# cfdeinza/reinforcement-learning-rendezvous

Measured on NVIDIA B200. Metric: env-steps/sec, higher is better.
Workload: dtype f64

## Files before the change

reinforcement_learning_rendezvous_b200/_native.py:

```python
from __future__ import annotations

import ctypes as C
import importlib.util
import os
import shutil
import subprocess
import sysconfig

PKG_DIR = os.path.dirname(os.path.abspath(__file__))
CSRC_DIR = os.path.join(PKG_DIR, "csrc")
INCLUDE_DIR = os.path.join(os.path.dirname(PKG_DIR), "include")
LIB_PATH = os.environ.get("RDV_B200_LIB") or os.path.join(CSRC_DIR, "librdv_b200.so")
HOST_SRC = os.path.join(CSRC_DIR, "rdv_host.c")
HOST_LIB = os.path.join(PKG_DIR, "_rdv_host" + (sysconfig.get_config_var("EXT_SUFFIX") or ".so"))
SOURCES = ("rdv_b200.cu",)
HEADERS = ("rdv_math.cuh", "rdv_env.cuh", "rdv_step.cuh", "rdv_policy.cuh", "rdv_policy_tc.cuh")

ABI_VERSION = 15
OBS_DIM, ACT_DIM, N_UNIFORMS = 17, 6, 24

(RCX, RCY, RCZ, VCX, VCY, VCZ, QCW, QCX, QCY, QCZ, WCX, WCY, WCZ, QTW, QTX, QTY, QTZ, WTX, WTY, WTZ,
 TDV, TDW, EPRET, NF64) = range(24)
I_STEP, I_SUCCESS, I_COLLIDED, I_EPISODE, NI32 = range(5)
STAT_NAMES = ("steps", "episodes", "return_sum", "length_sum", "succeeded", "collided", "delta_v_sum",
              "delta_w_sum", "end_obs", "end_time", "end_bubble", "end_attitude", "reward_sum",
              "rk_accepted", "rk_rejected", "failures")
NSTATS = len(STAT_NAMES)
EP_RETURN, EP_LENGTH, EP_SUCCESS, EP_COLLIDED, EP_DELTA_V, EP_DELTA_W, EP_NCOL = range(7)
INTEGRATOR_RK45, INTEGRATOR_CLOSED_FORM = 0, 1
END_REASONS = ("obs", "time", "bubble", "attitude")


class RdvParams(C.Structure):
    _fields_ = [
        ("rc0", C.c_double * 3), ("vc0", C.c_double * 3), ("qc0", C.c_double * 4),
        ("wc0", C.c_double * 3), ("qt0", C.c_double * 4), ("wt0", C.c_double * 3),
        ("rc0_range", C.c_double), ("vc0_range", C.c_double), ("qc0_range", C.c_double),
        ("wc0_range", C.c_double), ("qt0_range", C.c_double), ("wt0_range", C.c_double),
        ("koz_radius", C.c_double), ("corridor_half_angle", C.c_double), ("h", C.c_double),
        ("dt", C.c_double), ("t_max", C.c_double),
        ("collision_coef", C.c_double), ("bonus_coef", C.c_double), ("fuel_coef", C.c_double),
        ("att_coef", C.c_double),
        ("inertia_c", C.c_double * 9), ("inertia_t", C.c_double * 9),
        ("torque_c", C.c_double * 3),
        ("integrator", C.c_int32), ("reserved0", C.c_int32),
        ("inv_inertia_c", C.c_double * 9), ("inv_inertia_t", C.c_double * 9),
        ("max_delta_v", C.c_double), ("max_delta_w", C.c_double), ("max_axial_distance", C.c_double),
        ("max_axial_speed", C.c_double), ("max_wc", C.c_double),
        ("max_attitude_error", C.c_double), ("max_rd_error", C.c_double), ("max_vd_error", C.c_double),
        ("max_qd_error", C.c_double), ("max_wd_error", C.c_double),
        ("rd", C.c_double * 3), ("capture_axis", C.c_double * 3), ("corridor_axis", C.c_double * 3),
        ("bubble0", C.c_double), ("bubble_rate", C.c_double), ("bubble_min", C.c_double), ("n", C.c_double),
        ("cw", C.c_double * 17),
        ("max_delta_v_f32", C.c_float), ("fuel_num_f32", C.c_float), ("fuel_den_f32", C.c_float),
        ("iso_c", C.c_int32), ("iso_t", C.c_int32), ("done_steps", C.c_int32),
        ("inv_max_attitude_error", C.c_double), ("inv_max_rd_error", C.c_double), ("inv_max_qd_error", C.c_double),
        ("koz_radius_sq", C.c_double), ("max_rd_error_sq", C.c_double), ("max_vd_error_sq", C.c_double),
        ("max_wd_error_sq", C.c_double),
        ("fuel_scale", C.c_double),
        ("att_scale", C.c_double), ("bonus_scale", C.c_double), ("collision_scale", C.c_double),
        ("obs_inv_r", C.c_double), ("obs_inv_v", C.c_double), ("obs_inv_w", C.c_double),
        ("near_sq", C.c_double),
        ("box_hi_r", C.c_int32), ("box_hi_v", C.c_int32), ("box_hi_w", C.c_int32), ("reserved1", C.c_int32),
    ]


class RdvState(C.Structure):
    _fields_ = [("f64", C.c_void_p), ("i32", C.c_void_p), ("ld", C.c_int64), ("param_table", C.c_void_p),
                ("param_block", C.c_void_p)]


class RdvStepIO(C.Structure):
    _fields_ = [
        ("actions", C.c_void_p), ("act_f64", C.c_int32), ("auto_reset", C.c_int32),
        ("obs", C.c_void_p), ("reward", C.c_void_p), ("done", C.c_void_p),
        ("terminal_obs", C.c_void_p), ("end_reason", C.c_void_p), ("episode_record", C.c_void_p),
        ("stats", C.c_void_p),
        ("reward_f32", C.c_void_p), ("fin_count", C.c_void_p), ("fin_rows", C.c_void_p),
        ("fin_capacity", C.c_int32), ("fin_append", C.c_int32), ("fin_env_base", C.c_int32), ("reserved", C.c_int32),
    ]


class RdvFinishedRow(C.Structure):
    _fields_ = [("env", C.c_int32), ("end_reason", C.c_int32), ("terminal_obs", C.c_float * 17), ("pad", C.c_float),
                ("record", C.c_double * 6)]


class RdvPolicy(C.Structure):
    _fields_ = [
        ("w0", C.c_void_p), ("b0", C.c_void_p), ("w1", C.c_void_p), ("b1", C.c_void_p),
        ("w2", C.c_void_p), ("b2", C.c_void_p), ("hidden", C.c_int32), ("reserved", C.c_int32),
        ("log_std", C.c_void_p),
    ]


class RdvRolloutIO(C.Structure):
    _fields_ = [
        ("steps", C.c_int32), ("action_source", C.c_int32), ("auto_reset", C.c_int32), ("reserved", C.c_int32),
        ("actions", C.c_void_p), ("action_seed", C.c_uint64), ("step_base", C.c_int64),
        ("actions_out", C.c_void_p), ("obs", C.c_void_p), ("rewards", C.c_void_p), ("dones", C.c_void_p),
        ("obs_steps", C.c_void_p), ("stats", C.c_void_p), ("policy", RdvPolicy),
        ("reset_rows", C.c_void_p), ("sm_reserve", C.c_int32), ("reserved2", C.c_int32), ("mc_out", C.c_void_p),
    ]


RESET_ROWS = 23
(MC_EP_LEN, MC_NUM_COLLISIONS, MC_COLLIDED, MC_TOTAL_REWARD, MC_TOTAL_DELTA_V, MC_NUM_SUCCESSES, MC_SUCCEEDED,
 MC_MIN_KOZ, MC_POS_ERR, MC_VEL_ERR, MC_ATT_ERR, MC_ROT_ERR, MC_LEVEL, MC_TAIL_COUNT, MC_END_REASON,
 MC_TOTAL_DELTA_W, MC_NCOL) = range(17)
TUNE_ROLLOUT_TPB, TUNE_RESET_REFILL, TUNE_ROLLOUT_PDL, TUNE_ROLLOUT_HELPERS = 0, 1, 2, 3


ACTIONS_F32, ACTIONS_F64, ACTIONS_PHILOX, ACTIONS_POLICY, ACTIONS_POLICY_SAMPLE = 0, 1, 2, 3, 4


PROTOTYPES = {
    "rdv_abi_version": (C.c_int, []),
    "rdv_sizeof_params": (C.c_int, []),
    "rdv_sizeof": (C.c_int, [C.c_int]),
    "rdv_strerror": (C.c_char_p, [C.c_int]),
    "rdv_tune": (C.c_int, [C.c_int, C.c_int]),
    "rdv_params_default": (None, [C.POINTER(RdvParams)]),
    "rdv_params_derive": (C.c_int, [C.POINTER(RdvParams)]),
    "rdv_step": (C.c_int, [C.POINTER(RdvParams), C.POINTER(RdvState), C.POINTER(RdvStepIO), C.c_int64,
                           C.c_uint64, C.c_int64, C.c_void_p]),
    "rdv_rollout": (C.c_int, [C.POINTER(RdvParams), C.POINTER(RdvState), C.POINTER(RdvRolloutIO), C.c_int64,
                              C.c_uint64, C.c_int64, C.c_void_p]),
    "rdv_reset": (C.c_int, [C.POINTER(RdvParams), C.POINTER(RdvState), C.c_void_p, C.c_void_p, C.c_void_p,
                            C.c_int64, C.c_uint64, C.c_int64, C.c_int, C.c_void_p]),
    "rdv_observe": (C.c_int, [C.POINTER(RdvParams), C.POINTER(RdvState), C.c_void_p, C.c_int64, C.c_void_p]),
    "rdv_errors": (C.c_int, [C.POINTER(RdvParams), C.POINTER(RdvState), C.c_void_p, C.c_void_p, C.c_void_p,
                             C.c_void_p, C.c_int64, C.c_void_p]),
    "rdv_refresh_flags": (C.c_int, [C.POINTER(RdvParams), C.POINTER(RdvState), C.c_int64, C.c_void_p]),
    "rdv_frame_transform": (C.c_int, [C.c_void_p, C.c_void_p, C.c_void_p, C.c_int64, C.c_int, C.c_void_p]),
    "rdv_policy_forward": (C.c_int, [C.POINTER(RdvPolicy), C.c_void_p, C.c_void_p, C.c_int64, C.c_void_p]),
    "rdv_policy_forward_ffma": (C.c_int, [C.POINTER(RdvPolicy), C.c_void_p, C.c_void_p, C.c_int64, C.c_void_p]),
    "rdv_math_probe": (C.c_int, [C.c_void_p, C.c_void_p, C.c_int64, C.c_int, C.c_void_p]),
    "rdv_fp64_peak_probe": (C.c_int, [C.c_void_p, C.c_int, C.c_int, C.c_int, C.c_void_p]),
}

_lib = None


def nvcc_command(out=LIB_PATH):
    nvcc = shutil.which("nvcc") or "/usr/local/cuda/bin/nvcc"
    return [nvcc, "-gencode", "arch=compute_100a,code=sm_100a", "-lineinfo", "-O3", "-std=c++17",
            "-I", INCLUDE_DIR, "-shared", "-Xcompiler", "-fPIC", "-o", out] + \
           [os.path.join(CSRC_DIR, s) for s in SOURCES]


def is_stale():
    if not os.path.exists(LIB_PATH):
        return True
    t = os.path.getmtime(LIB_PATH)
    deps = [os.path.join(CSRC_DIR, f) for f in SOURCES + HEADERS] + [os.path.join(INCLUDE_DIR, "rdv_b200.h")]
    return any(os.path.getmtime(d) > t for d in deps if os.path.exists(d))


def build_host(force=False):
    global _host
    if force or not os.path.exists(HOST_LIB) or os.path.getmtime(HOST_LIB) < os.path.getmtime(HOST_SRC):
        cc = shutil.which("gcc") or shutil.which("cc") or "gcc"
        import numpy
        subprocess.run([cc, "-O2", "-fPIC", "-shared", "-Wall", "-I", sysconfig.get_paths()["include"],
                        "-I", numpy.get_include(), "-o", HOST_LIB, HOST_SRC], check=True)
        _host = None
    return HOST_LIB


_host = None


def host():
    global _host
    if _host is None:
        if not os.path.exists(HOST_LIB):
            raise RuntimeError(f"{HOST_LIB} is missing: build it with `python -c 'import __graft_entry__ as g; g.build()'`")
        spec = importlib.util.spec_from_file_location("_rdv_host", HOST_LIB)
        mod = importlib.util.module_from_spec(spec)
        spec.loader.exec_module(mod)
        _host = mod
    return _host


def build(force=False, verbose=False):
    global _lib
    build_host(force=force)
    if force or is_stale():
        cmd = nvcc_command()
        if verbose:
            cmd = cmd[:1] + ["-Xptxas", "-v"] + cmd[1:]
            print(" ".join(cmd))
        subprocess.run(cmd, check=True)
        _lib = None
    return LIB_PATH


def lib():
    global _lib
    if _lib is None:
        if not os.path.exists(LIB_PATH):
            raise RuntimeError(
                f"{LIB_PATH} is missing: build it with `python -c 'import __graft_entry__ as g; g.build()'` "
                "(nvcc, sm_100a).  This package has no CPU fallback.")
        L = C.CDLL(LIB_PATH)
        for name, (res, args) in PROTOTYPES.items():
            fn = getattr(L, name)
            fn.restype, fn.argtypes = res, args
        if L.rdv_abi_version() != ABI_VERSION:
            raise RuntimeError(f"librdv_b200.so ABI {L.rdv_abi_version()} != binding ABI {ABI_VERSION}; rebuild")
        for which, mirror in enumerate((RdvParams, RdvState, RdvStepIO, RdvRolloutIO, RdvPolicy, RdvFinishedRow)):
            if L.rdv_sizeof(which) != C.sizeof(mirror):
                raise RuntimeError(f"{mirror.__name__} layout mismatch between include/rdv_b200.h "
                                   f"({L.rdv_sizeof(which)} B) and _native.py ({C.sizeof(mirror)} B)")
        _lib = L
    return _lib


def strerror(status: int) -> str:
    return lib().rdv_strerror(int(status)).decode()


def check(status: int, what: str):
    if status != 0:
        raise RuntimeError(f"{what} failed: {strerror(status)} (status {status})")
```

reinforcement_learning_rendezvous_b200/csrc/rdv_b200.cu:

```cuda
#include <cuda_runtime.h>
#include <math.h>
#include <string.h>
#include <stdlib.h>
#include <atomic>
#include <mutex>
#include "rdv_step.cuh"
#include "rdv_policy.cuh"
#include "rdv_policy_tc.cuh"

namespace rdv {


RDV_DEV double warp_sum(double v)
{
#pragma unroll
    for (int o = 16; o > 0; o >>= 1) v += __shfl_xor_sync(0xffffffffu, v, o);
    return v;
}

struct StepStats {
    unsigned steps, episodes, succeeded, collided, end0, end1, end2, end3, rk_acc, rk_rej, fail;
    double ep_return, ep_length, delta_v, delta_w, reward;
};

template <int NWARPS>
RDV_DEV void reduce_stats(const StepStats &st, double *g_stats, double (*s_stats)[RDV_NSTATS])
{
    const unsigned full = 0xffffffffu;
    const int lane = threadIdx.x & 31, warp = threadIdx.x >> 5;
    double v[RDV_NSTATS];
    v[RDV_S_STEPS] = (double)__reduce_add_sync(full, st.steps);
    v[RDV_S_EPISODES] = (double)__reduce_add_sync(full, st.episodes);
    v[RDV_S_RK_ACCEPTED] = (double)__reduce_add_sync(full, st.rk_acc);
    v[RDV_S_RK_REJECTED] = (double)__reduce_add_sync(full, st.rk_rej);
    v[RDV_S_FAILURES] = (double)__reduce_add_sync(full, st.fail);
    v[RDV_S_REWARD] = warp_sum(st.reward);
    const bool any_done = v[RDV_S_EPISODES] > 0.0;
    if (any_done) {
        v[RDV_S_SUCCEEDED] = (double)__reduce_add_sync(full, st.succeeded);
        v[RDV_S_COLLIDED] = (double)__reduce_add_sync(full, st.collided);
#pragma unroll
        for (int k = 0; k < 4; ++k) v[RDV_S_END_OBS + k] = (double)__reduce_add_sync(full, (k==0?st.end0:k==1?st.end1:k==2?st.end2:st.end3));
        v[RDV_S_RETURN] = warp_sum(st.ep_return);
        v[RDV_S_LENGTH] = warp_sum(st.ep_length);
        v[RDV_S_DELTA_V] = warp_sum(st.delta_v);
        v[RDV_S_DELTA_W] = warp_sum(st.delta_w);
    } else {
        v[RDV_S_SUCCEEDED] = v[RDV_S_COLLIDED] = v[RDV_S_RETURN] = v[RDV_S_LENGTH] = 0.0;
        v[RDV_S_DELTA_V] = v[RDV_S_DELTA_W] = 0.0;
#pragma unroll
        for (int k = 0; k < 4; ++k) v[RDV_S_END_OBS + k] = 0.0;
    }
    if (lane == 0) {
#pragma unroll
        for (int k = 0; k < RDV_NSTATS; ++k) s_stats[warp][k] = v[k];
    }
    __syncthreads();
    if (threadIdx.x < RDV_NSTATS) {
        double acc = 0.0;
#pragma unroll
        for (int w = 0; w < NWARPS; ++w) acc += s_stats[w][threadIdx.x];
        if (acc != 0.0) atomicAdd(g_stats + threadIdx.x, acc);
    }
}

template <bool TABLE>
RDV_DEV const RdvParams &params_of(const RdvParams &Pc, const RdvState &S, const int64_t env)
{
    if constexpr (TABLE) return S.param_table[S.param_block[env >> 5]];
    else return Pc;
}

RDV_DEV double pair_swap(double v) { return __shfl_xor_sync(0xffffffffu, v, 1); }
RDV_DEV int pair_swap(int v) { return __shfl_xor_sync(0xffffffffu, v, 1); }

#ifndef RDV_STEP_MIN_CTAS
#define RDV_STEP_MIN_CTAS 4
#endif
#ifndef RDV_EPB
#define RDV_EPB 64
#endif
constexpr int EPB = RDV_EPB;
constexpr int TPB = 2 * EPB;

template <bool ISO, bool ACT_F64, bool CLOSED, bool TABLE = false>
__global__ void __launch_bounds__(TPB, RDV_STEP_MIN_CTAS) step_kernel(const __grid_constant__ RdvParams Pc, const RdvState S,
                                                      const RdvStepIO io, const int64_t n, const uint64_t seed,
                                                      const int64_t env_offset)
{
    __shared__ __align__(16) float s_obs[EPB * RDV_OBS_DIM];
    __shared__ double s_stats[TPB / 32][RDV_NSTATS];
    __shared__ double s_team[TPB / RDV_TEAM][RDV_TEAM_ROW];
    __shared__ int s_reset_idx[EPB];
    __shared__ int s_reset_n, s_fin_base;
    __shared__ double s_fin_rec[EPB][RDV_EP_NCOL];
    __shared__ int s_fin_reason[EPB];
    if (threadIdx.x == 0) s_reset_n = 0;
    __syncthreads();

    const int body = threadIdx.x & 1;
    const int64_t base = (int64_t)blockIdx.x * EPB;
    const int64_t i_raw = base + (threadIdx.x >> 1);
    const bool active = i_raw < n;
    const int64_t i = active ? i_raw : n - 1;
    const int64_t ld = S.ld;
    const double *f = S.f64 + i;
    StepStats st = {};
    const RdvParams &P = params_of<TABLE>(Pc, S, i);

    const int qrow = body ? RDV_QTW : RDV_QCW, wrow = body ? RDV_WTX : RDV_WCX;
    double y[7];
#pragma unroll
    for (int k = 0; k < 4; ++k) y[k] = f[(qrow + k) * ld];
#pragma unroll
    for (int k = 0; k < 3; ++k) y[4 + k] = f[(wrow + k) * ld];

    double act[3], total = f[(body ? RDV_TDV : RDV_TDW) * ld], fuel = 0.0;
    if (ACT_F64) {
        const double *ap = static_cast<const double *>(io.actions) + 6 * i + (body ? 0 : 3);
        const double a0 = ap[0], a1 = ap[1], a2 = ap[2];
        const double scale = body ? P.max_delta_v : P.max_delta_w;
        const double sum = fabs(a0) + fabs(a1) + fabs(a2);
        act[0] = a0 * scale; act[1] = a1 * scale; act[2] = a2 * scale;
        total += sum * scale;
        fuel = P.fuel_scale * sum;
    } else {
        const float *ap = static_cast<const float *>(io.actions) + 6 * i + (body ? 0 : 3);
        const float a0 = ap[0], a1 = ap[1], a2 = ap[2];
        const float sum = __fadd_rn(__fadd_rn(fabsf(a0), fabsf(a1)), fabsf(a2));
        if (body) {
            act[0] = (double)__fmul_rn(a0, P.max_delta_v_f32);
            act[1] = (double)__fmul_rn(a1, P.max_delta_v_f32);
            act[2] = (double)__fmul_rn(a2, P.max_delta_v_f32);
            total = (double)__fadd_rn((float)total, __fmul_rn(sum, P.max_delta_v_f32));
            fuel = (double)__fdiv_rn(__fmul_rn(P.fuel_num_f32, sum), P.fuel_den_f32);
        } else {
            act[0] = (double)a0 * P.max_delta_w; act[1] = (double)a1 * P.max_delta_w;
            act[2] = (double)a2 * P.max_delta_w;
            total += (double)sum * P.max_delta_w;
        }
    }

    double qo[4];
#pragma unroll
    for (int k = 0; k < 4; ++k) qo[k] = pair_swap(y[k]);
    double rc[3] = {0.0, 0.0, 0.0}, vc[3] = {0.0, 0.0, 0.0};
    if (body) {
        const Rot Rc_old = rot_from_quat(qo);
        double dv[3];
        rot_apply(Rc_old, act, dv);
        const double r0 = f[RDV_RCX * ld], r1 = f[RDV_RCY * ld], r2 = f[RDV_RCZ * ld];
        const double v0 = f[RDV_VCX * ld] + dv[0], v1 = f[RDV_VCY * ld] + dv[1], v2 = f[RDV_VCZ * ld] + dv[2];
        const double *c = P.cw;
        rc[0] = fma(c[2], v1, fma(c[1], v0, c[0] * r0));
        rc[1] = fma(c[6], v1, fma(c[5], v0, fma(c[3], r0, c[4] * r1)));
        rc[2] = fma(c[8], v2, c[7] * r2);
        vc[0] = fma(c[11], v1, fma(c[10], v0, c[9] * r0));
        vc[1] = fma(c[14], v1, fma(c[13], v0, c[12] * r0));
        vc[2] = fma(c[16], v2, c[15] * r2);
    } else {
        y[4] += act[0]; y[5] += act[1]; y[6] += act[2];
    }

    int rk_acc = 0, rk_rej = 0, fail = 0;
    if (CLOSED) {
        closed_form_attitude(y, P.dt);
    } else {
        BodyConst bc;
        bc.I = body ? P.inertia_t : P.inertia_c;
        bc.Iinv = body ? P.inv_inertia_t : P.inv_inertia_c;
        bc.tau = body ? c_zero3 : P.torque_c;
        const int k = ISO ? rk45_iso_plane(y, P.dt, rk_rej) : rk45_attitude<ISO>(y, P.dt, bc, rk_rej);
        if (k < 0) fail = 1; else rk_acc = k;
    }
    {
        const double r = fast_rsqrt(dot4(y, y));
#pragma unroll
        for (int k = 0; k < 4; ++k) y[k] *= r;
    }

    const Rot R = rot_from_quat(y);
    double wl[3];
    rot_apply(R, y + 4, wl);
    double got[3];
#pragma unroll
    for (int k = 0; k < 3; ++k) got[k] = pair_swap(body ? rc[k] : wl[k]);
    double part0, part1, part2;
    int col_now = 0;
    if (body) {
        double rd_l[3], vd_l[3], ax[3], d[3];
        rot_apply(R, P.rd, rd_l);
        cross3(wl, rd_l, vd_l);
#pragma unroll
        for (int k = 0; k < 3; ++k) d[k] = rc[k] - rd_l[k];
        part0 = dot3(d, d);
#pragma unroll
        for (int k = 0; k < 3; ++k) d[k] = vc[k] - vd_l[k];
        part1 = dot3(d, d);
#pragma unroll
        for (int k = 0; k < 3; ++k) d[k] = got[k] - wl[k];
        part2 = dot3(d, d);
        const double rc_sq = dot3(rc, rc);
        if (rc_sq < P.koz_radius_sq) {
            rot_apply(R, P.corridor_axis, ax);
            const double th = rounded_angle_from(dot3(rc, ax), rc_sq, dot3(ax, ax));
            col_now = th > P.corridor_half_angle ? 1 : 0;
        }
    } else {
        double cap[3];
        rot_apply(R, P.capture_axis, cap);
        const double rc_sq = dot3(got, got);
        part0 = rounded_angle_from(-dot3(got, cap), rc_sq, dot3(cap, cap));
        part1 = rc_sq;
        part2 = 0.0;
    }
    const double pos_sq = pair_swap(part0), vel_sq = pair_swap(part1), rot_sq = pair_swap(part2);
    const double fuel_t = pair_swap(fuel), total_t = pair_swap(total);
    const int col_t = pair_swap(col_now);

    float *o = s_obs + (threadIdx.x >> 1) * RDV_OBS_DIM;
    const ObsScale sc = obs_scale(P);
    bool in_box = true;
    if (body) {
#pragma unroll
        for (int k = 0; k < 3; ++k) {
            const float a = (float)fma(2.0 * (rc[k] + sc.hi_r), sc.inv_r, -1.0);
            const float b = (float)fma(2.0 * (vc[k] + sc.hi_v), sc.inv_v, -1.0);
            o[k] = a; o[3 + k] = b;
            in_box = in_box && a >= -1.0f && a <= 1.0f && b >= -1.0f && b <= 1.0f;
        }
#pragma unroll
        for (int k = 0; k < 4; ++k) {
            const float a = (float)y[k];
            o[13 + k] = a;
            in_box = in_box && a >= -1.0f && a <= 1.0f;
        }
    } else {
#pragma unroll
        for (int k = 0; k < 4; ++k) {
            const float a = (float)y[k];
            o[6 + k] = a;
            in_box = in_box && a >= -1.0f && a <= 1.0f;
        }
#pragma unroll
        for (int k = 0; k < 3; ++k) {
            const float a = (float)fma(2.0 * (y[4 + k] + sc.hi_w), sc.inv_w, -1.0);
            o[10 + k] = a;
            in_box = in_box && a >= -1.0f && a <= 1.0f;
        }
    }
    const int box_t = pair_swap((int)in_box);

    double *fw = S.f64 + i;
    if (active) {
#pragma unroll
        for (int k = 0; k < 4; ++k) fw[(qrow + k) * ld] = y[k];
#pragma unroll
        for (int k = 0; k < 3; ++k) fw[(wrow + k) * ld] = y[4 + k];
        fw[(body ? RDV_TDV : RDV_TDW) * ld] = total;
        if (body) {
#pragma unroll
            for (int k = 0; k < 3; ++k) { fw[(RDV_RCX + k) * ld] = rc[k]; fw[(RDV_VCX + k) * ld] = vc[k]; }
        }
    }
    st.rk_acc = active ? rk_acc : 0; st.rk_rej = active ? rk_rej : 0; st.fail = active ? fail : 0;

    int done = 0, fin_pos = 0;
    if (!body) {
        int step = S.i32[RDV_I_STEP * ld + i], success = S.i32[RDV_I_SUCCESS * ld + i];
        int collided = S.i32[RDV_I_COLLIDED * ld + i];
        double ep_ret = f[RDV_EPRET * ld];
        const double att = part0, rc_sq = part1;
        if (!collided) {
            collided = col_t;
            if (!collided && pos_sq <= P.max_rd_error_sq && vel_sq <= P.max_vd_error_sq && att <= P.max_qd_error &&
                rot_sq <= P.max_wd_error_sq)
                success += 1;
        }
        step += 1;
        const double bubble = fmax(fma(-(double)step, P.bubble_rate, P.bubble0), P.bubble_min);
        const bool c0 = !(in_box && box_t), c1 = step >= P.done_steps, c2 = rc_sq > bubble * bubble,
                   c3 = att > P.max_attitude_error;
        done = (c0 || c1 || c2 || c3) ? 1 : 0;
        const int reason = c0 ? 0 : c1 ? 1 : c2 ? 2 : c3 ? 3 : -1;
        double rew = P.att_scale * fma(-att, P.inv_max_attitude_error, 1.0);
        rew += fuel_t;
        if (col_t) rew -= P.collision_scale;
        if (rc_sq < P.koz_radius_sq && !collided && pos_sq < P.max_rd_error_sq) {
            rew += P.bonus_scale * fma(-fast_sqrt(pos_sq), P.inv_max_rd_error, 2.0);
            if (att < P.max_qd_error) rew += P.bonus_scale * fma(-att, P.inv_max_qd_error, 2.0);
        }
        ep_ret += rew;
        if (active) {
            io.reward[i] = rew;
            if (io.reward_f32) io.reward_f32[i] = (float)rew;
            io.done[i] = (uint8_t)done;
            if (io.end_reason) io.end_reason[i] = (int8_t)reason;
            st.steps = 1; st.reward = rew;
            fw[RDV_EPRET * ld] = ep_ret;
            S.i32[RDV_I_STEP * ld + i] = step; S.i32[RDV_I_SUCCESS * ld + i] = success;
            S.i32[RDV_I_COLLIDED * ld + i] = collided;
            if (done) {
                st.episodes = 1; st.succeeded = success > 0; st.collided = collided;
                st.end0 = reason == 0; st.end1 = reason == 1; st.end2 = reason == 2; st.end3 = reason == 3;
                st.ep_return = ep_ret; st.ep_length = (double)step; st.delta_v = total_t; st.delta_w = total;
                if (io.episode_record) {
                    double *rec = io.episode_record + RDV_EP_NCOL * i;
                    rec[RDV_EP_RETURN] = ep_ret; rec[RDV_EP_LENGTH] = (double)step;
                    rec[RDV_EP_SUCCESS] = (double)success; rec[RDV_EP_COLLIDED] = (double)collided;
                    rec[RDV_EP_DELTA_V] = total_t; rec[RDV_EP_DELTA_W] = total;
                }
                if (io.auto_reset || io.fin_rows) {
                    fin_pos = atomicAdd(&s_reset_n, 1);
                    s_reset_idx[fin_pos] = threadIdx.x >> 1;
                }
                if (io.fin_rows) {
                    double *fr = s_fin_rec[threadIdx.x >> 1];
                    fr[RDV_EP_RETURN] = ep_ret; fr[RDV_EP_LENGTH] = (double)step;
                    fr[RDV_EP_SUCCESS] = (double)success; fr[RDV_EP_COLLIDED] = (double)collided;
                    fr[RDV_EP_DELTA_V] = total_t; fr[RDV_EP_DELTA_W] = total;
                    s_fin_reason[threadIdx.x >> 1] = reason;
                }
            }
        }
    }

    __syncwarp();
    const int done_pair = __shfl_sync(0xffffffffu, done, (threadIdx.x & 31) & ~1);
    if (io.terminal_obs) {
        if (done_pair && active) {
            float *to = io.terminal_obs + RDV_OBS_DIM * i;
            for (int k = body; k < RDV_OBS_DIM; k += 2) to[k] = o[k];
        }
    }
    if (io.fin_rows) {
        __syncthreads();
        if (threadIdx.x == 0) s_fin_base = s_reset_n ? atomicAdd(io.fin_count, s_reset_n) : 0;
        __syncthreads();
        const int pos_pair = __shfl_sync(0xffffffffu, fin_pos, (threadIdx.x & 31) & ~1);
        const int slot = s_fin_base + pos_pair;
        if (done_pair && active && slot < io.fin_capacity) {
            RdvFinishedRow *fr = static_cast<RdvFinishedRow *>(io.fin_rows) + slot;
            if (!body) {
                fr->env = io.fin_env_base + (int32_t)i; fr->end_reason = s_fin_reason[threadIdx.x >> 1]; fr->pad = 0.0f;
#pragma unroll
                for (int k = 0; k < RDV_EP_NCOL; ++k) fr->record[k] = s_fin_rec[threadIdx.x >> 1][k];
            }
            for (int k = body; k < RDV_OBS_DIM; k += 2) fr->terminal_obs[k] = o[k];
        }
    }

    __syncthreads();
    if (io.auto_reset) {
        const int count = s_reset_n, team = threadIdx.x / RDV_TEAM;
        for (int b = 0; b < count; b += TPB / RDV_TEAM) {
            if (b + (team & ~3) >= count) break;
            const bool valid = b + team < count;
            const int local = valid ? s_reset_idx[b + team] : 0;
            const int64_t ie = base + local < n ? base + local : n - 1;
            team_reset(params_of<TABLE>(Pc, S, ie), S, seed, env_offset + ie, ie, valid, 1, nullptr, s_team[team],
                       s_obs + local * RDV_OBS_DIM);
        }
        __syncthreads();
    }

    {
        const int64_t rows = (n - base) < EPB ? (n - base) : EPB;
        const int total_f = (int)rows * RDV_OBS_DIM;
        float *dst = io.obs + base * RDV_OBS_DIM;
        const int nvec = total_f >> 2;
        const float4 *src4 = reinterpret_cast<const float4 *>(s_obs);
        float4 *dst4 = reinterpret_cast<float4 *>(dst);
        for (int k = threadIdx.x; k < nvec; k += TPB) dst4[k] = src4[k];
        for (int k = (nvec << 2) + threadIdx.x; k < total_f; k += TPB) dst[k] = s_obs[k];
    }
    if (io.stats) reduce_stats<TPB / 32>(st, io.stats, s_stats);
}

#ifndef RDV_SYNC_PERIOD
#define RDV_SYNC_PERIOD 8
#endif
#ifndef RDV_HELP_POST_PERIOD
#define RDV_HELP_POST_PERIOD 3
#endif
#ifndef RDV_HELP_IDLE_NS
#define RDV_HELP_IDLE_NS 500
#endif
#ifndef RDV_TMEM_STASH
#define RDV_TMEM_STASH 1
#endif
#ifndef RDV_TMEM_STASH_MAIN
#define RDV_TMEM_STASH_MAIN 1
#endif
#ifndef RDV_LOCKSTEP_MAX_TPB
#define RDV_LOCKSTEP_MAX_TPB 256
#endif
constexpr int RDV_NEXT_ROW = 22;
constexpr int RDV_ROW_TAG = 22;

RDV_DEV void take_reset_row(const double *rw, const int64_t rs, EnvRegs &e, EnvCounters &c)
{
#pragma unroll
    for (int j = 0; j < 3; ++j) { e.rc[j] = rw[(RDV_RCX + j) * rs]; e.vc[j] = rw[(RDV_VCX + j) * rs]; }
#pragma unroll
    for (int j = 0; j < 4; ++j) { e.qc[j] = rw[(RDV_QCW + j) * rs]; e.qt[j] = rw[(RDV_QTW + j) * rs]; }
#pragma unroll
    for (int j = 0; j < 3; ++j) { e.wc[j] = rw[(RDV_WCX + j) * rs]; e.wt[j] = rw[(RDV_WTX + j) * rs]; }
    c.collided = (int)rw[20 * rs]; c.success = (int)rw[21 * rs];
    c.step = 0; c.episode += 1; c.tdv = c.tdw = c.ep_ret = 0.0;
}

template <bool ISO, bool CLOSED, int TPB_, bool POLICY = false, bool MC = false, bool TABLE = false, bool OBS = POLICY,
          bool HELP = false>
__global__ void __launch_bounds__(TPB_ + (HELP ? 64 : 0), 1)
rollout_kernel(const __grid_constant__ RdvParams Pc, const RdvState S, const __grid_constant__ RdvRolloutIO io,
               const int64_t n, const uint64_t seed, const int64_t env_offset)
{
    static_assert(!HELP || (!POLICY && !MC && !TABLE && !OBS), "helper warps: plain variant only");
    constexpr int NW = TPB_ / 32;
    constexpr int NWT = NW + (HELP ? 2 : 0);
    extern __shared__ __align__(128) unsigned char dyn_smem[];
    tc::TileSmem *ts = reinterpret_cast<tc::TileSmem *>(dyn_smem);
    uint32_t tmem_all = 0, mma_phase = 0;
    if (POLICY) {
        asm volatile("griddepcontrol.wait;" ::: "memory");
        tmem_all = tc::tile_setup<TPB_>(io.policy, *ts);
    }
    constexpr bool main_stash = !POLICY && !MC && ISO && !CLOSED && (RDV_TMEM_STASH_MAIN != 0);
    __shared__ uint32_t s_tmem_base;
    if constexpr (main_stash) {
        if (threadIdx.x < 32) {
            asm volatile("tcgen05.alloc.cta_group::1.sync.aligned.shared::cta.b32 [%0], %1;"
                         :: "r"(tc::smem_u32(&s_tmem_base)), "r"(tc::TMEM_COLS) : "memory");
            asm volatile("tcgen05.relinquish_alloc_permit.cta_group::1.sync.aligned;" ::: "memory");
        }
        tc::tc_fence_before();
        __syncthreads();
        tc::tc_fence_after();
        tmem_all = s_tmem_base;
    }
    constexpr bool own_stage = !POLICY && OBS;
    __shared__ __align__(16) float s_obs[own_stage ? NW : 1][own_stage ? 32 * RDV_OBS_DIM : 4];
    __shared__ double s_stats[NWT][RDV_NSTATS];
    __shared__ double s_team_static[POLICY ? 1 : NWT][4][RDV_TEAM_ROW];
    __shared__ int s_row_ep[HELP ? NW : 1][32], s_ep_req[HELP ? NW : 1][32];
    __shared__ unsigned s_todo[HELP ? NW : 1];
    __shared__ unsigned s_cancel;
    __shared__ int s_inflight[2];
    __shared__ int s_ndone;
    const unsigned full = 0xffffffffu;
    const int lane = threadIdx.x & 31, warp = threadIdx.x >> 5;
    if constexpr (HELP) {
        if (threadIdx.x < NW) s_todo[threadIdx.x] = 0u;
        if (threadIdx.x == 0) { s_ndone = 0; s_cancel = 0u; s_inflight[0] = s_inflight[1] = 0; }
        __syncthreads();
    }
    const int src = io.action_source;
    const int64_t ld = S.ld;
    const bool persist = io.reset_rows != nullptr && io.auto_reset && !MC && io.reserved > 0;
    const int refill = (!MC && io.auto_reset && io.reserved > 0 && (persist || (!POLICY && io.steps >= 2 * io.reserved)))
                           ? io.reserved : 0;
    double *next_rows = reinterpret_cast<double *>(dyn_smem) + (size_t)warp * 32 * RDV_NEXT_ROW;
    float *obs_stage = POLICY ? reinterpret_cast<float *>(ts->al[warp >> 2]) + (warp & 3) * (32 * RDV_OBS_DIM)
                              : own_stage ? s_obs[own_stage ? warp : 0] : reinterpret_cast<float *>(next_rows);
    double (*s_team_w)[RDV_TEAM_ROW] =
        POLICY ? reinterpret_cast<double (*)[RDV_TEAM_ROW]>(reinterpret_cast<char *>(ts->al[warp >> 2]) +
                                                             4 * 32 * RDV_OBS_DIM * sizeof(float)) + (warp & 3) * 4
               : s_team_static[POLICY ? 0 : warp];
    static_assert(4 * 32 * RDV_OBS_DIM * sizeof(float) + 4 * 4 * RDV_TEAM_ROW * sizeof(double) <= sizeof(ts->al[0]),
                  "staging rows + team rows must fit the group's activation tile");
    constexpr bool want_obs = POLICY || OBS;
    const int64_t units = TABLE ? (n + 31) / 32 : n, unit = TABLE ? 32 : 1;
    const int64_t lo = unit * (units * (int64_t)blockIdx.x / gridDim.x);
    const int64_t hi_raw = unit * (units * ((int64_t)blockIdx.x + 1) / gridDim.x), hi = hi_raw < n ? hi_raw : n;
    const int64_t span = hi - lo;
    const int passes = (int)((span + TPB_ - 1) / TPB_);
    const int64_t chunk = TABLE ? TPB_ : (passes > 0 ? (span + passes - 1) / passes : 0);
    StepStats st = {};
    asm volatile("griddepcontrol.wait;" ::: "memory");
    asm volatile("griddepcontrol.launch_dependents;");

    if constexpr (HELP) {
        if (warp >= NW && passes > 0) {
            const RdvParams &P = Pc;
            const int h = warp - NW;
            for (;;) {
                bool worked = false;
                for (int ww = h; ww < NW; ww += 2) {
                    if (!*(volatile unsigned *)&s_todo[ww]) continue;
                    unsigned m = 0;
                    if (lane == 0) {
                        *(volatile int *)&s_inflight[h] = ww + 1;
                        __threadfence_block();
                        m = atomicExch(&s_todo[ww], 0u);
                    }
                    m = __shfl_sync(full, m, 0);
                    worked = true;
                    double *rows = reinterpret_cast<double *>(dyn_smem) + (size_t)ww * 32 * RDV_NEXT_ROW;
                    while (m && !((*(volatile unsigned *)&s_cancel >> ww) & 1u)) {
                        const int team = lane >> 3;
                        const unsigned src_bit = __fns(m, 0, team + 1);
                        const int src_lane = src_bit < 32 ? (int)src_bit : 0;
                        const int r_episode = *(volatile int *)&s_ep_req[ww][src_lane];
                        team_reset_core(P, seed, env_offset + lo + ww * 32 + src_lane, r_episode, nullptr,
                                        src_bit < 32 ? rows + src_lane * RDV_NEXT_ROW : s_team_w[team]);
                        __threadfence_block();
                        if (src_bit < 32 && (lane & 7) == 0) *(volatile int *)&s_row_ep[ww][src_lane] = r_episode;
#pragma unroll
                        for (int j = 0; j < 4; ++j) m &= m - 1;
                    }
                    __syncwarp();
                    __threadfence_block();
                    if (lane == 0) *(volatile int *)&s_inflight[h] = 0;
                }
                if (*(volatile int *)&s_ndone >= NW) break;
                if (!worked) __nanosleep(RDV_HELP_IDLE_NS);
            }
        }
    }

    for (int pass = 0; pass < ((HELP && warp >= NW) ? 0 : passes); ++pass) {
        const int64_t c_lo = lo + pass * chunk, c_hi = (c_lo + chunk < hi) ? c_lo + chunk : hi;
        const int64_t warp_base = c_lo + warp * 32;
        const int64_t i_raw = warp_base + lane;
        const bool active = i_raw < c_hi;
        const int64_t i = active ? i_raw : c_hi - 1;
        const int64_t env_id = env_offset + i;
        const int rows_w = (int)((c_hi - warp_base) < 32 ? ((c_hi - warp_base) > 0 ? (c_hi - warp_base) : 0) : 32);
        const RdvParams &P = params_of<TABLE>(Pc, S, i);

        EnvRegs e;
        EnvCounters c;
        load_env(S, i, e);
        load_counters(S, i, c);
        float ov[RDV_OBS_DIM];
        if (want_obs) make_obs(e, obs_scale(P), ov);
        unsigned fresh = 0;
        int countdown = HELP ? RDV_HELP_POST_PERIOD : refill;
        double *my_row = POLICY ? io.reset_rows + i : next_rows + lane * RDV_NEXT_ROW;
        const int64_t row_stride = POLICY ? ld : 1;
        if (persist) {
            const bool ok = active && io.reset_rows[RDV_ROW_TAG * ld + i] == (double)(c.episode + 1);
            fresh = __ballot_sync(full, ok);
            if (!POLICY && ok) {
#pragma unroll
                for (int j = 0; j < RDV_NEXT_ROW; ++j) my_row[j] = io.reset_rows[j * ld + i];
            }
            __syncwarp();
        }
        auto post_requests = [&]() {
            if constexpr (HELP) {
                const bool want = active && *(volatile int *)&s_row_ep[warp][lane] != c.episode + 1;
                if (want) s_ep_req[warp][lane] = c.episode + 1;
                const unsigned wm = __ballot_sync(full, want);
                __threadfence_block();
                if (lane == 0 && wm) atomicOr(&s_todo[warp], wm);
            }
        };
        if constexpr (HELP) {
            s_row_ep[warp][lane] = ((fresh >> lane) & 1u) ? c.episode + 1 : -1;
            __syncwarp();
            post_requests();
        }
        auto fill_rows = [&](unsigned todo) {
            while (todo) {
                const int team = lane >> 3;
                const unsigned src_bit = __fns(todo, 0, team + 1);
                const int src_lane = src_bit < 32 ? (int)src_bit : lane;
                const int64_t r_env = __shfl_sync(full, env_id, src_lane);
                const int r_episode = __shfl_sync(full, c.episode, src_lane) + 1;
                if (POLICY) {
                    double *tr = s_team_w[team];
                    team_reset_core(P, seed, r_env, r_episode, nullptr, tr);
                    if (src_bit < 32) {
                        double *dst = io.reset_rows + (r_env - env_offset);
                        for (int j = lane & 7; j < RDV_NEXT_ROW; j += 8) dst[j * ld] = tr[j];
                        if ((lane & 7) == 0) dst[RDV_ROW_TAG * ld] = (double)r_episode;
                    }
                    __syncwarp();
                } else {
                    team_reset_core(P, seed, r_env, r_episode, nullptr,
                                    src_bit < 32 ? next_rows + src_lane * RDV_NEXT_ROW : s_team_w[team]);
                }
#pragma unroll
                for (int j = 0; j < 4; ++j) todo &= todo - 1;
            }
        };

        McAcc mc;
        bool alive = true;
        int mc_reason = -1;
        if constexpr (MC) {
            mc_init(mc);
            EvalDetail d;
            eval_detail_of_state(P, e, d);
            mc_sample(P, d, c.collided, mc);
        }

        ActionTerms t;
        auto policy_action = [&](const int k) {
            const int64_t row = (int64_t)k * n + i;
            float a[RDV_ACT_DIM];
            const int g = threadIdx.x >> 7;
            tc::tile_forward(*ts, g, threadIdx.x & 127, TPB_ - 128 * g < 128 ? TPB_ - 128 * g : 128, ov,
                             tmem_all + (uint32_t)g * tc::GROUP_COLS, mma_phase, a, [] {});
            const bool sample = src == RDV_ACTIONS_POLICY_SAMPLE;
            if (sample) {
                float z[RDV_ACT_DIM];
                philox_normals(io.action_seed, env_id, io.step_base + k, z);
#pragma unroll
                for (int j = 0; j < RDV_ACT_DIM; ++j) a[j] = fmaf(ts->std[j], z[j], a[j]);
            }
            float ac[RDV_ACT_DIM];
#pragma unroll
            for (int j = 0; j < RDV_ACT_DIM; ++j) ac[j] = fminf(1.0f, fmaxf(-1.0f, a[j]));
            if (io.actions_out && active) {
                const float *rec = sample ? a : ac;
                float2 *op = reinterpret_cast<float2 *>(reinterpret_cast<float *>(io.actions_out) + 6 * row);
                op[0] = make_float2(rec[0], rec[1]); op[1] = make_float2(rec[2], rec[3]);
                op[2] = make_float2(rec[4], rec[5]);
            }
#pragma unroll
            for (int j = 0; j < RDV_ACT_DIM; ++j) a[j] = ac[j];
            if (!MC || alive) ingest_action_f32(P, a, c, t);
        };
        auto step_phase = [&](const int k) {
            const int64_t row = (int64_t)k * n + i;
            int rk_acc = 0, rk_rej = 0, fail = 0;
            StepResult r;
            if constexpr (MC) {
                r.rew = 0.0; r.done = 0; r.reason = -1;
                if (alive) {
                    env_advance<ISO, CLOSED, (TPB_ <= RDV_LOCKSTEP_MAX_TPB)>(P, e, t, rk_acc, rk_rej, fail);
                    EvalDetail d;
                    r = env_evaluate<true, true>(P, e, t.fuel, c, ov, &d);
                    mc_sample(P, d, c.collided, mc);
                    mc.total_reward += r.rew;
                    mc.len += 1;
                    if (r.done) { alive = false; mc_reason = r.reason; }
                }
            } else if constexpr ((POLICY && RDV_TMEM_STASH) || main_stash) {
                env_translate(P, e, t);
                const uint32_t lane_addr = tmem_all + (uint32_t)(threadIdx.x >> 7) * tc::GROUP_COLS +
                                           ((uint32_t)(threadIdx.x & 96) << 16);
                {
                    uint32_t w[48];
                    int q = 0;
                    auto put = [&](double v) { w[q++] = (uint32_t)__double2loint(v); w[q++] = (uint32_t)__double2hiint(v); };
#pragma unroll
                    for (int j = 0; j < 3; ++j) { put(e.rc[j]); put(e.vc[j]); }
                    put(c.tdv); put(c.tdw); put(c.ep_ret); put(t.fuel);
                    put(st.ep_return); put(st.ep_length); put(st.delta_v); put(st.delta_w); put(st.reward);
                    w[q++] = (uint32_t)c.step; w[q++] = (uint32_t)c.success; w[q++] = (uint32_t)c.collided;
                    w[q++] = (uint32_t)c.episode;
                    w[q++] = st.steps; w[q++] = st.episodes; w[q++] = st.succeeded; w[q++] = st.collided;
                    w[q++] = st.end0; w[q++] = st.end1; w[q++] = st.end2; w[q++] = st.end3;
                    w[q++] = st.rk_acc; w[q++] = st.rk_rej; w[q++] = st.fail;
                    while (q < 48) w[q++] = 0u;
                    tc::tmem_st16(lane_addr, reinterpret_cast<const uint32_t (&)[16]>(w[0]));
                    tc::tmem_st16(lane_addr + 16, reinterpret_cast<const uint32_t (&)[16]>(w[16]));
                    tc::tmem_st16(lane_addr + 32, reinterpret_cast<const uint32_t (&)[16]>(w[32]));
                    tc::tmem_st_wait();
                }
                env_attitude<ISO, CLOSED, (TPB_ <= RDV_LOCKSTEP_MAX_TPB)>(P, e, t, rk_acc, rk_rej, fail);
                {
                    uint32_t w[48];
                    tc::tmem_ld16_issue(lane_addr, reinterpret_cast<uint32_t (&)[16]>(w[0]));
                    tc::tmem_ld16_issue(lane_addr + 16, reinterpret_cast<uint32_t (&)[16]>(w[16]));
                    tc::tmem_ld16_issue(lane_addr + 32, reinterpret_cast<uint32_t (&)[16]>(w[32]));
                    tc::tmem_ld_wait(reinterpret_cast<uint32_t (&)[16]>(w[0]));
                    tc::tmem_ld_wait(reinterpret_cast<uint32_t (&)[16]>(w[16]));
                    tc::tmem_ld_wait(reinterpret_cast<uint32_t (&)[16]>(w[32]));
                    int q = 0;
                    auto get = [&]() { const double v = __hiloint2double((int)w[q + 1], (int)w[q]); q += 2; return v; };
#pragma unroll
                    for (int j = 0; j < 3; ++j) { e.rc[j] = get(); e.vc[j] = get(); }
                    c.tdv = get(); c.tdw = get(); c.ep_ret = get(); t.fuel = get();
                    st.ep_return = get(); st.ep_length = get(); st.delta_v = get(); st.delta_w = get(); st.reward = get();
                    c.step = (int)w[q++]; c.success = (int)w[q++]; c.collided = (int)w[q++]; c.episode = (int)w[q++];
                    st.steps = w[q++]; st.episodes = w[q++]; st.succeeded = w[q++]; st.collided = w[q++];
                    st.end0 = w[q++]; st.end1 = w[q++]; st.end2 = w[q++]; st.end3 = w[q++];
                    st.rk_acc = w[q++]; st.rk_rej = w[q++]; st.fail = w[q++];
                }
                r = env_evaluate<want_obs>(P, e, t.fuel, c, ov);
            } else {
                env_advance<ISO, CLOSED, (TPB_ <= RDV_LOCKSTEP_MAX_TPB)>(P, e, t, rk_acc, rk_rej, fail);
                r = env_evaluate<want_obs>(P, e, t.fuel, c, ov);
            }
            const bool done = r.done && active;
            if (active) {
                if (io.rewards) io.rewards[row] = r.rew;
                if (io.dones) io.dones[row] = (uint8_t)r.done;
                if (!MC || r.reason != -1 || alive) {
                    st.steps += 1; st.reward += r.rew; st.rk_acc += rk_acc; st.rk_rej += rk_rej; st.fail += fail;
                }
                if (r.done) {
                    st.episodes += 1; st.succeeded += c.success > 0; st.collided += c.collided;
                    st.end0 += r.reason == 0; st.end1 += r.reason == 1; st.end2 += r.reason == 2;
                    st.end3 += r.reason == 3;
                    st.ep_return += c.ep_ret; st.ep_length += (double)c.step; st.delta_v += c.tdv; st.delta_w += c.tdw;
                }
            }
            if constexpr (HELP) {
                const unsigned m = __ballot_sync(full, done);
                if (m) {
                    const bool have = done && *(volatile int *)&s_row_ep[warp][lane] == c.episode + 1;
                    unsigned need = m & ~__ballot_sync(full, have);
                    if (have) {
                        __threadfence_block();
                        take_reset_row(my_row, 1, e, c);
                    }
                    while (need) {
                        const int team = lane >> 3;
                        const unsigned src_bit = __fns(need, 0, team + 1);
                        const int src_lane = src_bit < 32 ? (int)src_bit : lane;
                        const int64_t r_env = __shfl_sync(full, env_id, src_lane);
                        const int r_episode = __shfl_sync(full, c.episode, src_lane) + 1;
                        team_reset_core(P, seed, r_env, r_episode, nullptr, s_team_w[team]);
                        const int rank = __popc(need & ((1u << lane) - 1));
                        if (((need >> lane) & 1u) && rank < 4) take_reset_row(s_team_w[rank], 1, e, c);
                        __syncwarp();
#pragma unroll
                        for (int j = 0; j < 4; ++j) need &= need - 1;
                    }
                }
                if (--countdown <= 0) {
                    countdown = RDV_HELP_POST_PERIOD;
                    post_requests();
                }
            } else if (!MC && io.auto_reset && refill) {
                const unsigned m = __ballot_sync(full, done);
                const unsigned need = m & ~fresh;
                if (need) fill_rows(need);
                if (done) {
                    take_reset_row(my_row, row_stride, e, c);
                    if (want_obs) make_obs(e, obs_scale(P), ov);
                }
                fresh = (fresh | need) & ~m;
                __syncwarp();
                if (--countdown == 0 && k + 1 < io.steps) {
                    countdown = refill;
                    const unsigned todo = __ballot_sync(full, active) & ~fresh;
                    fill_rows(todo);
                    fresh |= todo;
                }
            } else if (!MC && io.auto_reset) {
                unsigned m = __ballot_sync(full, done);
                while (m) {
                    const int team = lane >> 3;
                    const unsigned src_bit = __fns(m, 0, team + 1);
                    const int src_lane = src_bit < 32 ? (int)src_bit : lane;
                    const int64_t r_env = __shfl_sync(full, env_id, src_lane);
                    const int r_episode = __shfl_sync(full, c.episode, src_lane) + 1;
                    team_reset_core(P, seed, r_env, r_episode, nullptr, s_team_w[team]);
                    const int rank = __popc(m & ((1u << lane) - 1));
                    if (((m >> lane) & 1u) && rank < 4) {
                        take_reset_row(s_team_w[rank], 1, e, c);
                        if (want_obs) make_obs(e, obs_scale(P), ov);
                    }
                    __syncwarp();
#pragma unroll
                    for (int j = 0; j < 4; ++j) m &= m - 1;
                }
            }
            if (want_obs && io.obs_steps) {
                float *o = obs_stage + lane * RDV_OBS_DIM;
#pragma unroll
                for (int j = 0; j < RDV_OBS_DIM; ++j) o[j] = ov[j];
                __syncwarp();
                float *dst = io.obs_steps + ((int64_t)k * n + warp_base) * RDV_OBS_DIM;
                for (int j = lane; j < rows_w * RDV_OBS_DIM; j += 32) dst[j] = obs_stage[j];
                __syncwarp();
            }
        };

        if constexpr (POLICY) {
            for (int k = 0; k < io.steps; ++k) {
                __syncthreads();
                policy_action(k);
                step_phase(k);
            }
        } else {
            for (int k = 0; k < io.steps; ++k) {
#if RDV_SYNC_PERIOD >= 1
                if ((k % RDV_SYNC_PERIOD) == 0) {
                    if constexpr (HELP) asm volatile("bar.sync 2, %0;" :: "n"(TPB_) : "memory");
                    else __syncthreads();
                }
#endif
                const int64_t row = (int64_t)k * n + i;
                if (src == RDV_ACTIONS_F32) {
                    const float2 *ap = reinterpret_cast<const float2 *>(static_cast<const float *>(io.actions) + 6 * row);
                    const float2 a01 = ap[0], a23 = ap[1], a45 = ap[2];
                    const float a[6] = {a01.x, a01.y, a23.x, a23.y, a45.x, a45.y};
                    if (!MC || alive) ingest_action_f32(P, a, c, t);
                } else {
                    double a[6];
                    if (src == RDV_ACTIONS_F64) {
                        const double2 *ap = reinterpret_cast<const double2 *>(static_cast<const double *>(io.actions) + 6 * row);
                        const double2 a01 = ap[0], a23 = ap[1], a45 = ap[2];
                        a[0] = a01.x; a[1] = a01.y; a[2] = a23.x; a[3] = a23.y; a[4] = a45.x; a[5] = a45.y;
                    } else {
                        philox_actions(io.action_seed, env_id, io.step_base + k, a);
                        if (io.actions_out && active) {
                            double2 *op = reinterpret_cast<double2 *>(io.actions_out + 6 * row);
                            op[0] = make_double2(a[0], a[1]); op[1] = make_double2(a[2], a[3]);
                            op[2] = make_double2(a[4], a[5]);
                        }
                    }
                    if (!MC || alive) ingest_action_f64(P, a, c, t);
                }
                step_phase(k);
            }
        }

        if constexpr (HELP) {
            if (lane == 0) {
                atomicOr(&s_cancel, 1u << warp);
                atomicExch(&s_todo[warp], 0u);
                __threadfence_block();
                while (*(volatile int *)&s_inflight[warp & 1] == warp + 1) { }
                atomicAdd(&s_ndone, 1);
            }
            __syncwarp();
            __threadfence_block();
            fresh = __ballot_sync(full, active && *(volatile int *)&s_row_ep[warp][lane] == c.episode + 1);
        }
        if (persist) {
            const unsigned todo = HELP ? 0u : __ballot_sync(full, active) & ~fresh;
            fill_rows(todo);
            if (!POLICY && active) {
                const bool ready = !HELP || ((fresh >> lane) & 1u);
                if (ready) {
#pragma unroll
                    for (int j = 0; j < RDV_NEXT_ROW; ++j) io.reset_rows[j * ld + i] = my_row[j];
                }
                io.reset_rows[RDV_ROW_TAG * ld + i] = ready ? (double)(c.episode + 1) : -1.0;
            }
            __syncwarp();
        }
        if (active) {
            store_env(S, i, e);
            store_counters(S, i, c);
            if constexpr (MC) {
                double *mo = io.mc_out + (size_t)RDV_MC_NCOL * i;
                const double inv = 1.0 / (double)(mc.count > 0 ? mc.count : 1);
                mo[RDV_MC_EP_LEN] = (double)mc.len; mo[RDV_MC_NUM_COLLISIONS] = (double)mc.n_col;
                mo[RDV_MC_COLLIDED] = mc.n_col > 0 ? 1.0 : 0.0; mo[RDV_MC_TOTAL_REWARD] = mc.total_reward;
                mo[RDV_MC_TOTAL_DELTA_V] = c.tdv; mo[RDV_MC_NUM_SUCCESSES] = (double)mc.n_suc;
                mo[RDV_MC_SUCCEEDED] = mc.n_suc > 0 ? 1.0 : 0.0; mo[RDV_MC_MIN_KOZ] = mc.min_koz;
                mo[RDV_MC_POS_ERR] = mc.sum[0] * inv; mo[RDV_MC_VEL_ERR] = mc.sum[1] * inv;
                mo[RDV_MC_ATT_ERR] = mc.sum[2] * inv; mo[RDV_MC_ROT_ERR] = mc.sum[3] * inv;
                mo[RDV_MC_LEVEL] = (double)mc.level; mo[RDV_MC_TAIL_COUNT] = (double)mc.count;
                mo[RDV_MC_END_REASON] = (double)mc_reason; mo[RDV_MC_TOTAL_DELTA_W] = c.tdw;
            }
        }
        if (!want_obs || MC) make_obs(e, obs_scale(P), ov);
        float *o = obs_stage + lane * RDV_OBS_DIM;
#pragma unroll
        for (int j = 0; j < RDV_OBS_DIM; ++j) o[j] = ov[j];
        __syncwarp();
        float *dst = io.obs + warp_base * RDV_OBS_DIM;
        for (int j = lane; j < rows_w * RDV_OBS_DIM; j += 32) dst[j] = obs_stage[j];
        __syncwarp();
    }
    if (io.stats) reduce_stats<NWT>(st, io.stats, s_stats);
    if (POLICY || main_stash) tc::tile_teardown(tmem_all);
}

template <bool TABLE>
__global__ void __launch_bounds__(128) reset_kernel(const __grid_constant__ RdvParams Pc, const RdvState S,
                                                    const uint8_t *mask, const double *uniforms, float *obs,
                                                    int64_t n, uint64_t seed, int64_t env_offset, int bump)
{
    __shared__ double s_team[128 / RDV_TEAM][RDV_TEAM_ROW];
    const int team = threadIdx.x / RDV_TEAM;
    const int64_t i_raw = (int64_t)blockIdx.x * (128 / RDV_TEAM) + team;
    const int64_t i = i_raw < n ? i_raw : n - 1;
    const bool valid = i_raw < n && (!mask || mask[i]);
    team_reset(params_of<TABLE>(Pc, S, i), S, seed, env_offset + i, i, valid, bump, uniforms ? uniforms + RDV_N_UNIFORMS * i : nullptr,
               s_team[team], obs ? obs + RDV_OBS_DIM * i : nullptr);
}

template <bool TABLE>
__global__ void __launch_bounds__(128) observe_kernel(const __grid_constant__ RdvParams Pc, const RdvState S,
                                                      float *obs, int64_t n)
{
    const int64_t i = (int64_t)blockIdx.x * blockDim.x + threadIdx.x;
    if (i >= n) return;
    const RdvParams &P = params_of<TABLE>(Pc, S, i);
    EnvRegs e;
    load_env(S, i, e);
    float ov[RDV_OBS_DIM];
    make_obs(e, obs_scale(P), ov);
#pragma unroll
    for (int k = 0; k < RDV_OBS_DIM; ++k) obs[RDV_OBS_DIM * i + k] = ov[k];
}

template <bool TABLE>
__global__ void __launch_bounds__(128) errors_kernel(const __grid_constant__ RdvParams Pc, const RdvState S,
                                                     double *errors, uint8_t *collision, uint8_t *success,
                                                     double *koz, int64_t n, int refresh_flags)
{
    const int64_t i = (int64_t)blockIdx.x * blockDim.x + threadIdx.x;
    if (i >= n) return;
    const RdvParams &P = params_of<TABLE>(Pc, S, i);
    EnvRegs e;
    load_env(S, i, e);
    const Rot Rc = rot_from_quat(e.qc), Rt = rot_from_quat(e.qt);
    const double rc_sq = dot3(e.rc, e.rc), rc_n = sqrt(rc_sq);
    const double att = attitude_error(P, e, Rc, rc_sq);
    const double th = corridor_angle(P, e, Rt, rc_sq);
    const bool col = rc_n < P.koz_radius && th > P.corridor_half_angle;
    ErrSq es = errors_sq(P, e, Rc, Rt);
    const double pe = sqrt(es.pos), ve = sqrt(es.vel), re = sqrt(es.rot);
    const bool within = pe <= P.max_rd_error && ve <= P.max_vd_error && att <= P.max_qd_error && re <= P.max_wd_error;
    if (refresh_flags) {
        S.i32[RDV_I_COLLIDED * S.ld + i] = col ? 1 : 0;
        S.i32[RDV_I_SUCCESS * S.ld + i] = (!col && within) ? 1 : 0;
        return;
    }
    const int sticky = S.i32[RDV_I_COLLIDED * S.ld + i];
    if (errors) { errors[4 * i] = pe; errors[4 * i + 1] = ve; errors[4 * i + 2] = att; errors[4 * i + 3] = re; }
    if (collision) collision[i] = col ? 1 : 0;
    if (success) success[i] = (!sticky && within) ? 1 : 0;
    if (koz) koz[i] = koz_distance(P, rc_n, th);
}

__global__ void __launch_bounds__(128) frame_kernel(const double *q, const double *v, double *out, int64_t n,
                                                    int transpose)
{
    const int64_t i = (int64_t)blockIdx.x * blockDim.x + threadIdx.x;
    if (i >= n) return;
    const double qq[4] = {q[4 * i], q[4 * i + 1], q[4 * i + 2], q[4 * i + 3]};
    const double vv[3] = {v[3 * i], v[3 * i + 1], v[3 * i + 2]};
    double o[3];
    const Rot R = rot_from_quat(qq);
    if (transpose) rot_apply_T(R, vv, o); else rot_apply(R, vv, o);
    out[3 * i] = o[0]; out[3 * i + 1] = o[1]; out[3 * i + 2] = o[2];
}

constexpr int PH = 64;
constexpr int PTPB = 128;
__global__ void __launch_bounds__(PTPB) policy_kernel(const RdvPolicy pi, const float *obs, float *actions, int64_t n)
{
    extern __shared__ __align__(16) float sm[];
    float *w0 = sm, *w1 = w0 + PH * 17, *w2 = w1 + PH * PH, *b0 = w2 + 6 * PH, *b1 = b0 + PH, *b2 = b1 + PH;
    float *hid = b2 + 8;
    for (int k = threadIdx.x; k < PH * 17; k += PTPB) w0[k] = pi.w0[k];
    for (int k = threadIdx.x; k < PH * PH; k += PTPB) w1[k] = pi.w1[k];
    for (int k = threadIdx.x; k < 6 * PH; k += PTPB) w2[k] = pi.w2[k];
    for (int k = threadIdx.x; k < PH; k += PTPB) { b0[k] = pi.b0[k]; b1[k] = pi.b1[k]; }
    if (threadIdx.x < 6) b2[threadIdx.x] = pi.b2[threadIdx.x];
    __syncthreads();
    const int64_t i = (int64_t)blockIdx.x * PTPB + threadIdx.x;
    if (i >= n) return;
    float x[17];
#pragma unroll
    for (int k = 0; k < 17; ++k) x[k] = obs[17 * i + k];
    float h[PH];
#pragma unroll
    for (int j = 0; j < PH; ++j) {
        float acc = b0[j];
#pragma unroll
        for (int k = 0; k < 17; ++k) acc = fmaf(w0[j * 17 + k], x[k], acc);
        h[j] = tanhf(acc);
    }
#pragma unroll 1
    for (int j = 0; j < PH; ++j) {
        float acc = b1[j];
        const float4 *wr = reinterpret_cast<const float4 *>(w1 + j * PH);
#pragma unroll
        for (int k4 = 0; k4 < PH / 4; ++k4) {
            float4 w = wr[k4];
            acc = fmaf(w.x, h[4 * k4], acc); acc = fmaf(w.y, h[4 * k4 + 1], acc);
            acc = fmaf(w.z, h[4 * k4 + 2], acc); acc = fmaf(w.w, h[4 * k4 + 3], acc);
        }
        hid[j * PTPB + threadIdx.x] = tanhf(acc);
    }
#pragma unroll
    for (int k = 0; k < PH; ++k) h[k] = hid[k * PTPB + threadIdx.x];
#pragma unroll
    for (int j = 0; j < 6; ++j) {
        float acc = b2[j];
#pragma unroll
        for (int k = 0; k < PH; ++k) acc = fmaf(w2[j * PH + k], h[k], acc);
        actions[6 * i + j] = fminf(1.0f, fmaxf(-1.0f, acc));
    }
}

__global__ void math_probe_kernel(const double *x, double *y, int64_t n, int op)
{
    const int64_t i = (int64_t)blockIdx.x * blockDim.x + threadIdx.x;
    if (i >= n) return;
    const double v = x[i];
    double r;
    switch (op) {
        case 0: r = fast_rsqrt(v); break;
        case 1: r = fast_rcp(v); break;
        case 2: r = fast_sqrt(v); break;
        case 3: r = pow_neg_tenth(v); break;
        case 4: r = (double)pow_neg_tenth_f32((float)v); break;
        default: r = rounded_angle_from(v, 1.0, 1.0); break;
    }
    y[i] = r;
}

__global__ void fp64_peak_kernel(double *sink, int iters)
{
    double a[16];
#pragma unroll
    for (int k = 0; k < 16; ++k) a[k] = 1.0 + 1e-9 * (threadIdx.x + k);
    const double m = 1.0 + 1e-12 * threadIdx.x, c = 1e-15;
    for (int it = 0; it < iters; ++it) {
#pragma unroll
        for (int k = 0; k < 16; ++k) a[k] = fma(a[k], m, c);
    }
    double s = 0.0;
#pragma unroll
    for (int k = 0; k < 16; ++k) s += a[k];
    sink[(size_t)blockIdx.x * blockDim.x + threadIdx.x] = s;
}

}

using namespace rdv;

static int check_state(const RdvState *s, int64_t n)
{
    if (!s || !s->f64 || !s->i32) return RDV_ERR_NULL;
    if (n < 0 || s->ld < n) return RDV_ERR_SIZE;
    if (((uintptr_t)s->f64 & 7) || ((uintptr_t)s->i32 & 3)) return RDV_ERR_ALIGN;
    if (s->param_table && !s->param_block) return RDV_ERR_NULL;
    if (((uintptr_t)s->param_table & 7) || ((uintptr_t)s->param_block & 3)) return RDV_ERR_ALIGN;
    return RDV_OK;
}
static int launch_status()
{
    cudaError_t e = cudaGetLastError();
    return e == cudaSuccess ? RDV_OK : RDV_ERR_CUDA;
}

constexpr int RDV_MAX_DEVICES = 64;
static std::atomic<int> g_sm_count[RDV_MAX_DEVICES];
static int current_device(int *sm_count)
{
    int dev = 0;
    if (cudaGetDevice(&dev) != cudaSuccess || dev < 0 || dev >= RDV_MAX_DEVICES) return -1;
    int sms = g_sm_count[dev].load(std::memory_order_relaxed);
    if (sms == 0) {
        if (cudaDeviceGetAttribute(&sms, cudaDevAttrMultiProcessorCount, dev) != cudaSuccess || sms <= 0) return -1;
        g_sm_count[dev].store(sms, std::memory_order_relaxed);
    }
    *sm_count = sms;
    return dev;
}
template <class K>
static bool ensure_smem(K kernel, std::atomic<uint64_t> &mask, int dev, size_t bytes)
{
    const uint64_t bit = 1ull << dev;
    if (mask.load(std::memory_order_acquire) & bit) return true;
    if (cudaFuncSetAttribute(kernel, cudaFuncAttributeMaxDynamicSharedMemorySize, (int)bytes) != cudaSuccess) return false;
    mask.fetch_or(bit, std::memory_order_release);
    return true;
}

#if RDV_ACOS_TABLE
__global__ void acos_table_kernel()
{
    const int i = blockIdx.x * blockDim.x + threadIdx.x;
    if (i <= 2 * ACOS_TABLE_HALF) g_acos_table[i] = acos_of_rounded((double)(i - ACOS_TABLE_HALF));
}
#endif
static bool ensure_tables(cudaStream_t st)
{
#if RDV_ACOS_TABLE
    static std::atomic<uint64_t> mask{0};
    static std::mutex mtx;
    int dev = 0;
    if (cudaGetDevice(&dev) != cudaSuccess || dev < 0 || dev >= RDV_MAX_DEVICES) return false;
    const uint64_t bit = 1ull << dev;
    if (mask.load(std::memory_order_acquire) & bit) return true;
    std::lock_guard<std::mutex> lock(mtx);
    if (mask.load(std::memory_order_acquire) & bit) return true;
    cudaStreamCaptureStatus cap = cudaStreamCaptureStatusNone;
    if (cudaStreamIsCapturing(st, &cap) != cudaSuccess || cap != cudaStreamCaptureStatusNone) return false;
    acos_table_kernel<<<(2 * ACOS_TABLE_HALF + 256) / 256, 256, 0, st>>>();
    if (cudaGetLastError() != cudaSuccess || cudaStreamSynchronize(st) != cudaSuccess) return false;
    mask.fetch_or(bit, std::memory_order_release);
#else
    (void)st;
#endif
    return true;
}

static int env_int(const char *name, int fallback)
{
    const char *v = getenv(name);
    return v ? atoi(v) : fallback;
}
static std::atomic<int> g_tune_tpb{env_int("RDV_ROLLOUT_TPB", 0)};
static std::atomic<int> g_tune_refill{env_int("RDV_RESET_REFILL", 12)};
static std::atomic<int> g_tune_pdl{env_int("RDV_ROLLOUT_PDL", 1)};
static std::atomic<int> g_tune_helpers{env_int("RDV_ROLLOUT_HELPERS", 1)};

extern "C" {

int rdv_abi_version(void) { return RDV_ABI_VERSION; }

int rdv_tune(int key, int value)
{
    if (key == RDV_TUNE_ROLLOUT_TPB) return g_tune_tpb.exchange(value);
    if (key == RDV_TUNE_RESET_REFILL) return g_tune_refill.exchange(value);
    if (key == RDV_TUNE_ROLLOUT_PDL) return g_tune_pdl.exchange(value);
    if (key == RDV_TUNE_ROLLOUT_HELPERS) return g_tune_helpers.exchange(value);
    return RDV_ERR_SIZE;
}
int rdv_sizeof_params(void) { return (int)sizeof(RdvParams); }
int rdv_sizeof(int which)
{
    switch (which) {
        case 0: return (int)sizeof(RdvParams);
        case 1: return (int)sizeof(RdvState);
        case 2: return (int)sizeof(RdvStepIO);
        case 3: return (int)sizeof(RdvRolloutIO);
        case 4: return (int)sizeof(RdvPolicy);
        case 5: return (int)sizeof(RdvFinishedRow);
        default: return -1;
    }
}

const char *rdv_strerror(int status)
{
    switch (status) {
        case RDV_OK: return "ok";
        case RDV_ERR_NULL: return "required pointer is NULL";
        case RDV_ERR_SIZE: return "bad size, leading dimension or enum value";
        case RDV_ERR_ALIGN: return "pointer not aligned for vector access";
        case RDV_ERR_PARAMS: return "invalid environment parameters";
        case RDV_ERR_CUDA: return "CUDA launch/runtime failure (is a B200 visible?)";
        case RDV_ERR_UNSUPPORTED: return "unsupported configuration";
        default: return "unknown status";
    }
}

void rdv_params_default(RdvParams *p)
{
    memset(p, 0, sizeof(*p));
    const double rad = M_PI / 180.0;
    p->rc0[1] = -10.0; p->qc0[0] = 1.0; p->qt0[0] = 1.0;
    p->rc0_range = 1; p->vc0_range = 0.1; p->qc0_range = 1 * rad; p->wc0_range = 0.1 * rad;
    p->qt0_range = 45 * rad; p->wt0_range = 3 * rad;
    p->koz_radius = 5; p->corridor_half_angle = 30 * rad; p->h = 800e3; p->dt = 1; p->t_max = 120;
    p->collision_coef = 0.5; p->bonus_coef = 8; p->fuel_coef = 0.2; p->att_coef = 1;
    const double diag = 1.0 * 1 / 12 * 100 * 2;
    for (int i = 0; i < 3; ++i) { p->inertia_c[4 * i] = diag; p->inertia_t[4 * i] = diag; }
    p->integrator = RDV_INTEGRATOR_RK45;
}

static int invert3(const double *m, double *o)
{
    double c00 = m[4] * m[8] - m[5] * m[7], c01 = m[5] * m[6] - m[3] * m[8], c02 = m[3] * m[7] - m[4] * m[6];
    double det = m[0] * c00 + m[1] * c01 + m[2] * c02;
    if (!(fabs(det) > 0.0)) return -1;
    bool diag = m[1] == 0 && m[2] == 0 && m[3] == 0 && m[5] == 0 && m[6] == 0 && m[7] == 0;
    if (diag) {
        for (int i = 0; i < 9; ++i) o[i] = 0.0;
        o[0] = 1.0 / m[0]; o[4] = 1.0 / m[4]; o[8] = 1.0 / m[8];
        return 0;
    }
    o[0] = c00 / det; o[1] = (m[2] * m[7] - m[1] * m[8]) / det; o[2] = (m[1] * m[5] - m[2] * m[4]) / det;
    o[3] = c01 / det; o[4] = (m[0] * m[8] - m[2] * m[6]) / det; o[5] = (m[2] * m[3] - m[0] * m[5]) / det;
    o[6] = c02 / det; o[7] = (m[1] * m[6] - m[0] * m[7]) / det; o[8] = (m[0] * m[4] - m[1] * m[3]) / det;
    return 0;
}
static int is_isotropic(const double *m, const double *tau)
{
    bool off = m[1] == 0 && m[2] == 0 && m[3] == 0 && m[5] == 0 && m[6] == 0 && m[7] == 0;
    bool eq = m[0] == m[4] && m[4] == m[8];
    bool t0 = !tau || (tau[0] == 0 && tau[1] == 0 && tau[2] == 0);
    return off && eq && t0;
}

int rdv_params_derive(RdvParams *p)
{
    if (!p) return RDV_ERR_NULL;
    const double rad = M_PI / 180.0;
    const double nominal_diag = 1.0 * 1 / 12 * 100 * 2;
    if (invert3(p->inertia_c, p->inv_inertia_c) || invert3(p->inertia_t, p->inv_inertia_t)) return RDV_ERR_PARAMS;
    p->max_delta_v = 10.0 / 100 * 0.5;
    p->max_delta_w = 0.2 / nominal_diag * 0.5;
    p->max_axial_distance = sqrt(p->rc0[0] * p->rc0[0] + p->rc0[1] * p->rc0[1] + p->rc0[2] * p->rc0[2]) + 10;
    p->max_axial_speed = 5; p->max_wc = 10 * rad; p->max_attitude_error = 30 * rad;
    p->max_rd_error = 0.5; p->max_vd_error = 0.1; p->max_qd_error = 5 * rad; p->max_wd_error = 1 * rad;
    p->rd[0] = 0; p->rd[1] = -2; p->rd[2] = 0;
    p->capture_axis[0] = 0; p->capture_axis[1] = 1; p->capture_axis[2] = 0;
    p->corridor_axis[0] = 0; p->corridor_axis[1] = -1; p->corridor_axis[2] = 0;
    p->bubble0 = p->max_axial_distance;
    p->bubble_rate = 0.5 * p->dt;
    const double rd_n = 2.0;
    p->bubble_min = rd_n + 2 * p->max_rd_error;
    const double ro = 6371e3 + p->h;
    p->n = sqrt(3.986004418e14 / (ro * ro * ro));
    if (!(rd_n < p->koz_radius) || !(rd_n - p->max_rd_error > 0)) return RDV_ERR_PARAMS;
    if (!(p->dt > 0) || !(p->t_max > 0)) return RDV_ERR_PARAMS;
    if (fabs(p->dt * 1000.0 - rint(p->dt * 1000.0)) > 1e-9 * p->dt * 1000.0) return RDV_ERR_UNSUPPORTED;
    const double n = p->n, nt = n * p->dt, s = sin(nt), c = cos(nt);
    double *w = p->cw;
    w[0] = 4 - 3 * c;          w[1] = 1 / n * s;            w[2] = 2 / n * (1 - c);
    w[3] = 6 * (s - nt);       w[4] = 1;                    w[5] = -2 / n * (1 - c);  w[6] = 1 / n * (4 * s - 3 * nt);
    w[7] = c;                  w[8] = 1 / n * s;
    w[9] = 3 * n * s;          w[10] = c;                   w[11] = 2 * s;
    w[12] = -6 * n * (1 - c);  w[13] = -2 * s;              w[14] = 4 * c - 3;
    w[15] = -n * s;            w[16] = c;
    p->max_delta_v_f32 = (float)p->max_delta_v;
    p->fuel_num_f32 = (float)(p->dt * p->fuel_coef);
    p->fuel_den_f32 = (float)(3 * p->max_delta_v);
    p->inv_max_attitude_error = 1.0 / p->max_attitude_error;
    p->inv_max_rd_error = 1.0 / p->max_rd_error;
    p->inv_max_qd_error = 1.0 / p->max_qd_error;
    p->koz_radius_sq = p->koz_radius * p->koz_radius;
    p->max_rd_error_sq = p->max_rd_error * p->max_rd_error;
    p->max_vd_error_sq = p->max_vd_error * p->max_vd_error;
    p->max_wd_error_sq = p->max_wd_error * p->max_wd_error;
    p->fuel_scale = p->dt * p->fuel_coef / (3 * p->max_delta_v);
    p->att_scale = p->dt * p->att_coef;
    p->bonus_scale = p->dt * p->bonus_coef;
    p->collision_scale = p->dt * p->collision_coef;
    p->obs_inv_r = 1.0 / (2.0 * p->max_axial_distance);
    p->obs_inv_v = 1.0 / (2.0 * p->max_axial_speed);
    p->obs_inv_w = 1.0 / (2.0 * p->max_wc);
    {
        auto hiword = [](double x) { uint64_t b; memcpy(&b, &x, 8); return (int32_t)((b >> 32) & 0x7fffffffu); };
        p->box_hi_r = hiword(p->max_axial_distance * (1.0 - 1e-6));
        p->box_hi_v = hiword(p->max_axial_speed * (1.0 - 1e-6));
        p->box_hi_w = hiword(p->max_wc * (1.0 - 1e-6));
        p->reserved1 = 0;
    }
    {
        const double reach = rd_n + p->max_rd_error, lim = reach > p->koz_radius ? reach : p->koz_radius;
        p->near_sq = lim * lim * (1.0 + 1e-9);
    }
    {
        double k = ceil(p->t_max / p->dt) - 2.0;
        if (k < 1.0) k = 1.0;
        while (rint(k * p->dt * 1000.0) / 1000.0 < p->t_max) k += 1.0;
        if (k > 2147483647.0) return RDV_ERR_PARAMS;
        p->done_steps = (int32_t)k;
    }
    p->iso_c = is_isotropic(p->inertia_c, p->torque_c);
    p->iso_t = is_isotropic(p->inertia_t, nullptr);
    if (p->integrator != RDV_INTEGRATOR_RK45 && p->integrator != RDV_INTEGRATOR_CLOSED_FORM) return RDV_ERR_SIZE;
    if (p->integrator == RDV_INTEGRATOR_CLOSED_FORM && !(p->iso_c && p->iso_t)) return RDV_ERR_UNSUPPORTED;
    return RDV_OK;
}

int rdv_step(const RdvParams *p, const RdvState *s, const RdvStepIO *io, int64_t n, uint64_t seed,
             int64_t env_offset, void *cuda_stream)
{
    if (!p || !io || !io->actions || !io->obs || !io->reward || !io->done) return RDV_ERR_NULL;
    int rc = check_state(s, n);
    if (rc) return rc;
    if (n == 0) return RDV_OK;
    if (((uintptr_t)io->actions & (io->act_f64 ? 15 : 7)) || ((uintptr_t)io->obs & 15) || ((uintptr_t)io->reward & 7))
        return RDV_ERR_ALIGN;
    cudaStream_t st = (cudaStream_t)cuda_stream;
    const unsigned grid = (unsigned)((n + EPB - 1) / EPB);
    const bool iso = p->iso_c && p->iso_t;
    const bool closed = p->integrator == RDV_INTEGRATOR_CLOSED_FORM;
    if (io->auto_reset != 0 && io->auto_reset != 1) return RDV_ERR_SIZE;
    if (io->fin_rows) {
        if (!io->fin_count) return RDV_ERR_NULL;
        if (io->fin_capacity < 0) return RDV_ERR_SIZE;
        if (((uintptr_t)io->fin_rows & 15) || ((uintptr_t)io->fin_count & 3)) return RDV_ERR_ALIGN;
        if (!io->fin_append && cudaMemsetAsync(io->fin_count, 0, sizeof(int32_t), st) != cudaSuccess) return RDV_ERR_CUDA;
    }
    if ((uintptr_t)io->reward_f32 & 3) return RDV_ERR_ALIGN;
    if (!ensure_tables(st)) return RDV_ERR_CUDA;
#define RDV_LAUNCH(ISO_, F64_, CL_) \
    step_kernel<ISO_, F64_, CL_><<<grid, TPB, 0, st>>>(*p, *s, *io, n, seed, env_offset)
    if (s->param_table) {
        if (!iso || closed) return RDV_ERR_UNSUPPORTED;
        if (io->act_f64) step_kernel<true, true, false, true><<<grid, TPB, 0, st>>>(*p, *s, *io, n, seed, env_offset);
        else step_kernel<true, false, false, true><<<grid, TPB, 0, st>>>(*p, *s, *io, n, seed, env_offset);
    }
    else if (closed) { if (io->act_f64) RDV_LAUNCH(true, true, true); else RDV_LAUNCH(true, false, true); }
    else if (iso) { if (io->act_f64) RDV_LAUNCH(true, true, false); else RDV_LAUNCH(true, false, false); }
    else { if (io->act_f64) RDV_LAUNCH(false, true, false); else RDV_LAUNCH(false, false, false); }
#undef RDV_LAUNCH
    return launch_status();
}

int rdv_rollout(const RdvParams *p, const RdvState *s, const RdvRolloutIO *io, int64_t n, uint64_t seed,
                int64_t env_offset, void *cuda_stream)
{
    if (!p || !io || !io->obs) return RDV_ERR_NULL;
    int rc = check_state(s, n);
    if (rc) return rc;
    if (io->steps < 0 || io->action_source < 0 || io->action_source > RDV_ACTIONS_POLICY_SAMPLE) return RDV_ERR_SIZE;
    if (io->auto_reset != 0 && io->auto_reset != 1) return RDV_ERR_SIZE;
    const bool policy = io->action_source == RDV_ACTIONS_POLICY || io->action_source == RDV_ACTIONS_POLICY_SAMPLE;
    if (policy) {
        const RdvPolicy *pi = &io->policy;
        if (io->action_source == RDV_ACTIONS_POLICY_SAMPLE && !pi->log_std) return RDV_ERR_NULL;
        if (!pi->w0 || !pi->b0 || !pi->w1 || !pi->b1 || !pi->w2 || !pi->b2) return RDV_ERR_NULL;
        if (pi->hidden != PI_H) return RDV_ERR_UNSUPPORTED;
    } else if (io->action_source != RDV_ACTIONS_PHILOX && !io->actions) return RDV_ERR_NULL;
    if (((uintptr_t)io->actions & (io->action_source == RDV_ACTIONS_F64 ? 15 : 7)) || ((uintptr_t)io->actions_out & 15) ||
        ((uintptr_t)io->obs & 3) || ((uintptr_t)io->rewards & 7))
        return RDV_ERR_ALIGN;
    if (n == 0 || io->steps == 0) return RDV_OK;
    cudaStream_t st = (cudaStream_t)cuda_stream;
    const bool iso = p->iso_c && p->iso_t;
    const bool closed = p->integrator == RDV_INTEGRATOR_CLOSED_FORM;
    int sm_count = 0;
    const int dev = current_device(&sm_count);
    if (dev < 0 || !ensure_tables(st)) return RDV_ERR_CUDA;
    if (io->sm_reserve < 0 || io->sm_reserve >= sm_count) return RDV_ERR_SIZE;
    const int64_t sms = sm_count - io->sm_reserve;
    const int64_t grid = n < sms ? n : sms;
    const int64_t per_cta = (n + grid - 1) / grid;
    const bool mc = io->mc_out != nullptr;
    if (mc && (io->auto_reset || ((uintptr_t)io->mc_out & 7))) return io->auto_reset ? RDV_ERR_UNSUPPORTED : RDV_ERR_ALIGN;
    if ((uintptr_t)io->reset_rows & 7) return RDV_ERR_ALIGN;
    const bool table = s->param_table != nullptr;
    const int force_tpb = (mc || table) ? 256 : g_tune_tpb.load(std::memory_order_relaxed);
    const int64_t max_tpb = force_tpb > 0 ? force_tpb : 512;
    const int64_t passes = (per_cta + max_tpb - 1) / max_tpb;
    const int64_t chunk = force_tpb > 0 ? force_tpb : (per_cta + passes - 1) / passes;
    RdvRolloutIO io_k = *io;
    io_k.reserved = g_tune_refill.load(std::memory_order_relaxed);
    if (io_k.reserved < 0 || io_k.reserved > 64) io_k.reserved = 0;
#define RDV_LAUNCH_K(KERNEL, T_, SMEM)                                                                            \
    {                                                                                                             \
        static std::atomic<uint64_t> attr_mask{0};                                                                \
        if (!ensure_smem(KERNEL, attr_mask, dev, SMEM)) return RDV_ERR_CUDA;                                      \
        if (g_tune_pdl.load(std::memory_order_relaxed)) {                                                         \
            cudaLaunchConfig_t cfg = {};                                                                          \
            cfg.gridDim = dim3((unsigned)grid); cfg.blockDim = dim3(T_); cfg.dynamicSmemBytes = SMEM; cfg.stream = st; \
            cudaLaunchAttribute at[1];                                                                            \
            at[0].id = cudaLaunchAttributeProgrammaticStreamSerialization;                                        \
            at[0].val.programmaticStreamSerializationAllowed = 1;                                                 \
            cfg.attrs = at; cfg.numAttrs = 1;                                                                     \
            if (cudaLaunchKernelEx(&cfg, KERNEL, *p, *s, io_k, n, seed, env_offset) != cudaSuccess) {             \
                cudaGetLastError();                                                                               \
                return RDV_ERR_CUDA;                                                                              \
            }                                                                                                     \
        } else {                                                                                                  \
            KERNEL<<<(unsigned)grid, T_, SMEM, st>>>(*p, *s, io_k, n, seed, env_offset);                          \
        }                                                                                                         \
    }
#define RDV_ROWS_SMEM(T_) ((size_t)(T_ / 32) * 32 * RDV_NEXT_ROW * sizeof(double))
#define RDV_LAUNCH_R(ISO_, CL_, T_) RDV_LAUNCH_K((rollout_kernel<ISO_, CL_, T_, false, false>), T_, RDV_ROWS_SMEM(T_))
#define RDV_LAUNCH_OBS(ISO_, CL_) \
    RDV_LAUNCH_K((rollout_kernel<ISO_, CL_, 256, false, false, false, true>), 256, RDV_ROWS_SMEM(256))
    const bool helpers = g_tune_helpers.load(std::memory_order_relaxed) && io->auto_reset && io_k.reserved > 0 &&
                         (io_k.reset_rows != nullptr || io->steps >= 2 * io_k.reserved) &&
                         passes == 1 && chunk > 384 && chunk <= 448;
#define RDV_LAUNCH_H(ISO_, CL_) \
    RDV_LAUNCH_K((rollout_kernel<ISO_, CL_, 448, false, false, false, false, true>), 512, RDV_ROWS_SMEM(448))
#define RDV_PICK_R(ISO_, CL_)                                 \
    if (io->obs_steps) RDV_LAUNCH_OBS(ISO_, CL_)              \
    else if (chunk <= 256) RDV_LAUNCH_R(ISO_, CL_, 256)       \
    else if (chunk <= 384) RDV_LAUNCH_R(ISO_, CL_, 384)       \
    else if (chunk <= 448) { if (helpers && ISO_ && !CL_) RDV_LAUNCH_H(true, false) else RDV_LAUNCH_R(ISO_, CL_, 448) } \
    else RDV_LAUNCH_R(ISO_, CL_, 512)
#define RDV_LAUNCH_P(T_) RDV_LAUNCH_K((rollout_kernel<true, false, T_, true, false>), T_, sizeof(tc::TileSmem))
    if (table) {
        if (!iso || closed) return RDV_ERR_UNSUPPORTED;
        if (mc && policy) RDV_LAUNCH_K((rollout_kernel<true, false, 256, true, true, true>), 256, sizeof(tc::TileSmem))
        else if (mc) RDV_LAUNCH_K((rollout_kernel<true, false, 256, false, true, true, true>), 256, RDV_ROWS_SMEM(256))
        else if (policy) RDV_LAUNCH_K((rollout_kernel<true, false, 256, true, false, true>), 256, sizeof(tc::TileSmem))
        else RDV_LAUNCH_K((rollout_kernel<true, false, 256, false, false, true, true>), 256, RDV_ROWS_SMEM(256))
    }
    else if (mc) {
        if (!iso || closed) return RDV_ERR_UNSUPPORTED;
        if (policy) RDV_LAUNCH_K((rollout_kernel<true, false, 256, true, true>), 256, sizeof(tc::TileSmem))
        else RDV_LAUNCH_K((rollout_kernel<true, false, 256, false, true, false, true>), 256, RDV_ROWS_SMEM(256))
    }
    else if (policy) {
        if (!iso || closed) return RDV_ERR_UNSUPPORTED;
        if (chunk <= 256) RDV_LAUNCH_P(256)
        else if (chunk <= 384) RDV_LAUNCH_P(384)
        else if (chunk <= 448) RDV_LAUNCH_P(448)
        else RDV_LAUNCH_P(512)
    }
    else if (closed) { RDV_PICK_R(true, true) }
    else if (iso) { RDV_PICK_R(true, false) }
    else RDV_LAUNCH_OBS(false, false)
#undef RDV_LAUNCH_OBS
#undef RDV_LAUNCH_P
#undef RDV_PICK_R
#undef RDV_LAUNCH_H
#undef RDV_LAUNCH_R
#undef RDV_ROWS_SMEM
#undef RDV_LAUNCH_K
    return launch_status();
}

int rdv_reset(const RdvParams *p, const RdvState *s, const uint8_t *mask, const double *uniforms, float *obs,
              int64_t n, uint64_t seed, int64_t env_offset, int bump_episode, void *cuda_stream)
{
    if (!p) return RDV_ERR_NULL;
    int rc = check_state(s, n);
    if (rc) return rc;
    if (n == 0) return RDV_OK;
    const int64_t per_cta = 128 / RDV_TEAM;
    const unsigned grid = (unsigned)((n + per_cta - 1) / per_cta);
    if (s->param_table)
        reset_kernel<true><<<grid, 128, 0, (cudaStream_t)cuda_stream>>>(*p, *s, mask, uniforms, obs, n, seed, env_offset,
                                                                        bump_episode ? 1 : 0);
    else
        reset_kernel<false><<<grid, 128, 0, (cudaStream_t)cuda_stream>>>(*p, *s, mask, uniforms, obs, n, seed, env_offset,
                                                                         bump_episode ? 1 : 0);
    return launch_status();
}

int rdv_observe(const RdvParams *p, const RdvState *s, float *obs, int64_t n, void *cuda_stream)
{
    if (!p || !obs) return RDV_ERR_NULL;
    int rc = check_state(s, n);
    if (rc) return rc;
    if (n == 0) return RDV_OK;
    if (s->param_table) observe_kernel<true><<<(unsigned)((n + 127) / 128), 128, 0, (cudaStream_t)cuda_stream>>>(*p, *s, obs, n);
    else observe_kernel<false><<<(unsigned)((n + 127) / 128), 128, 0, (cudaStream_t)cuda_stream>>>(*p, *s, obs, n);
    return launch_status();
}

int rdv_errors(const RdvParams *p, const RdvState *s, double *errors, uint8_t *collision, uint8_t *success,
               double *koz, int64_t n, void *cuda_stream)
{
    if (!p) return RDV_ERR_NULL;
    int rc = check_state(s, n);
    if (rc) return rc;
    if (n == 0) return RDV_OK;
    if (!ensure_tables((cudaStream_t)cuda_stream)) return RDV_ERR_CUDA;
    if (s->param_table)
        errors_kernel<true><<<(unsigned)((n + 127) / 128), 128, 0, (cudaStream_t)cuda_stream>>>(*p, *s, errors, collision,
                                                                                                 success, koz, n, 0);
    else
        errors_kernel<false><<<(unsigned)((n + 127) / 128), 128, 0, (cudaStream_t)cuda_stream>>>(*p, *s, errors, collision,
                                                                                                  success, koz, n, 0);
    return launch_status();
}

int rdv_refresh_flags(const RdvParams *p, const RdvState *s, int64_t n, void *cuda_stream)
{
    if (!p) return RDV_ERR_NULL;
    int rc = check_state(s, n);
    if (rc) return rc;
    if (n == 0) return RDV_OK;
    if (!ensure_tables((cudaStream_t)cuda_stream)) return RDV_ERR_CUDA;
    if (s->param_table)
        errors_kernel<true><<<(unsigned)((n + 127) / 128), 128, 0, (cudaStream_t)cuda_stream>>>(*p, *s, nullptr, nullptr,
                                                                                                 nullptr, nullptr, n, 1);
    else
        errors_kernel<false><<<(unsigned)((n + 127) / 128), 128, 0, (cudaStream_t)cuda_stream>>>(*p, *s, nullptr, nullptr,
                                                                                                  nullptr, nullptr, n, 1);
    return launch_status();
}

int rdv_frame_transform(const double *q, const double *v, double *out, int64_t n, int transpose, void *cuda_stream)
{
    if (!q || !v || !out) return RDV_ERR_NULL;
    if (n < 0) return RDV_ERR_SIZE;
    if (n == 0) return RDV_OK;
    frame_kernel<<<(unsigned)((n + 127) / 128), 128, 0, (cudaStream_t)cuda_stream>>>(q, v, out, n, transpose);
    return launch_status();
}

int rdv_policy_forward(const RdvPolicy *pi, const float *obs, float *actions, int64_t n, void *cuda_stream)
{
    if (!pi || !obs || !actions || !pi->w0 || !pi->b0 || !pi->w1 || !pi->b1 || !pi->w2 || !pi->b2) return RDV_ERR_NULL;
    if (pi->hidden != tc::H) return RDV_ERR_UNSUPPORTED;
    if (n < 0) return RDV_ERR_SIZE;
    if (n == 0) return RDV_OK;
    int sm_count = 0;
    const int dev = current_device(&sm_count);
    if (dev < 0) return RDV_ERR_CUDA;
    static std::atomic<uint64_t> attr_mask{0};
    if (!ensure_smem(tc::policy_tc_kernel, attr_mask, dev, sizeof(tc::Smem))) return RDV_ERR_CUDA;
    const int64_t tiles = (n + tc::TM - 1) / tc::TM;
    const unsigned grid = (unsigned)(tiles < sm_count ? tiles : sm_count);
    tc::policy_tc_kernel<<<grid, tc::GROUPS * tc::TM, sizeof(tc::Smem), (cudaStream_t)cuda_stream>>>(*pi, obs, actions, n);
    return launch_status();
}

int rdv_policy_forward_ffma(const RdvPolicy *pi, const float *obs, float *actions, int64_t n, void *cuda_stream)
{
    if (!pi || !obs || !actions || !pi->w0 || !pi->b0 || !pi->w1 || !pi->b1 || !pi->w2 || !pi->b2) return RDV_ERR_NULL;
    if (pi->hidden != PH) return RDV_ERR_UNSUPPORTED;
    if (n < 0) return RDV_ERR_SIZE;
    if (n == 0) return RDV_OK;
    const size_t smem = sizeof(float) * (PH * 17 + PH * PH + 6 * PH + PH + PH + 8 + PH * PTPB);
    int sm_count = 0;
    const int dev = current_device(&sm_count);
    if (dev < 0) return RDV_ERR_CUDA;
    static std::atomic<uint64_t> attr_mask{0};
    if (!ensure_smem(policy_kernel, attr_mask, dev, smem)) return RDV_ERR_CUDA;
    policy_kernel<<<(unsigned)((n + PTPB - 1) / PTPB), PTPB, smem, (cudaStream_t)cuda_stream>>>(*pi, obs, actions, n);
    return launch_status();
}

int rdv_math_probe(const double *x, double *y, int64_t n, int op, void *cuda_stream)
{
    if (!x || !y) return RDV_ERR_NULL;
    if (n < 0 || op < 0 || op > 5) return RDV_ERR_SIZE;
    if (n == 0) return RDV_OK;
    if (!ensure_tables((cudaStream_t)cuda_stream)) return RDV_ERR_CUDA;
    math_probe_kernel<<<(unsigned)((n + 255) / 256), 256, 0, (cudaStream_t)cuda_stream>>>(x, y, n, op);
    return launch_status();
}

int rdv_fp64_peak_probe(double *sink, int blocks, int threads, int iters, void *cuda_stream)
{
    if (!sink) return RDV_ERR_NULL;
    if (blocks <= 0 || threads <= 0 || threads > 1024 || iters <= 0) return RDV_ERR_SIZE;
    fp64_peak_kernel<<<blocks, threads, 0, (cudaStream_t)cuda_stream>>>(sink, iters);
    return launch_status();
}

}
```

reinforcement_learning_rendezvous_b200/csrc/rdv_math.cuh:

```cuda
#pragma once
#include <cuda_runtime.h>
#include <stdint.h>
#include "rdv_b200.h"

#define RDV_DEV __device__ __forceinline__

namespace rdv {

RDV_DEV double fast_rcp(double x)
{
    double r;
    asm("rcp.approx.ftz.f64 %0, %1;" : "=d"(r) : "d"(x));
    double e = fma(-x, r, 1.0);
    r = fma(r, e, r);
    e = fma(-x, r, 1.0);
    r = fma(r, e, r);
    return r;
}

RDV_DEV double fast_rsqrt(double x)
{
    double r;
    asm("rsqrt.approx.ftz.f64 %0, %1;" : "=d"(r) : "d"(x));
    const double m = x * r;
    const double e = fma(-m, r, 1.0);
    const double p = fma(0.375, e, 0.5);
    return fma(r * e, p, r);
}

RDV_DEV double pow_neg_tenth(double x)
{
    if (!(x >= 1e-30 && x <= 1e30)) return pow(x, -0.1);
    float lf = __log2f((float)x);
    double y = (double)exp2f(-0.1f * lf);
#pragma unroll
    for (int it = 0; it < 2; ++it) {
        double y2 = y * y, y4 = y2 * y2, y8 = y4 * y4, y10 = y8 * y2;
        double res = fma(-x, y10, 1.0);
        y = fma(y * 0.1, res, y);
    }
    return y;
}

RDV_DEV double dot3(const double a[3], const double b[3]) { return fma(a[2], b[2], fma(a[1], b[1], a[0] * b[0])); }
RDV_DEV double dot4(const double a[4], const double b[4])
{
    return fma(a[3], b[3], fma(a[2], b[2], fma(a[1], b[1], a[0] * b[0])));
}
RDV_DEV void cross3(const double a[3], const double b[3], double o[3])
{
    o[0] = fma(a[1], b[2], -(a[2] * b[1]));
    o[1] = fma(a[2], b[0], -(a[0] * b[2]));
    o[2] = fma(a[0], b[1], -(a[1] * b[0]));
}

struct Rot { double m[9]; };
RDV_DEV Rot rot_from_quat(const double q_in[4])
{
    double r = fast_rsqrt(dot4(q_in, q_in));
    double w = q_in[0] * r, x = q_in[1] * r, y = q_in[2] * r, z = q_in[3] * r;
    double ww = w * w;
    Rot R;
    R.m[0] = fma(2.0, fma(x, x, ww), -1.0); R.m[1] = 2.0 * fma(x, y, -(w * z)); R.m[2] = 2.0 * fma(x, z, w * y);
    R.m[3] = 2.0 * fma(x, y, w * z); R.m[4] = fma(2.0, fma(y, y, ww), -1.0); R.m[5] = 2.0 * fma(y, z, -(w * x));
    R.m[6] = 2.0 * fma(x, z, -(w * y)); R.m[7] = 2.0 * fma(y, z, w * x); R.m[8] = fma(2.0, fma(z, z, ww), -1.0);
    return R;
}
RDV_DEV Rot rot_from_unit_quat(const double q[4])
{
    const double w = q[0], x = q[1], y = q[2], z = q[3];
    const double ww = w * w;
    Rot R;
    R.m[0] = fma(2.0, fma(x, x, ww), -1.0); R.m[1] = 2.0 * fma(x, y, -(w * z)); R.m[2] = 2.0 * fma(x, z, w * y);
    R.m[3] = 2.0 * fma(x, y, w * z); R.m[4] = fma(2.0, fma(y, y, ww), -1.0); R.m[5] = 2.0 * fma(y, z, -(w * x));
    R.m[6] = 2.0 * fma(x, z, -(w * y)); R.m[7] = 2.0 * fma(y, z, w * x); R.m[8] = fma(2.0, fma(z, z, ww), -1.0);
    return R;
}
RDV_DEV void rot_apply(const Rot &R, const double v[3], double o[3])
{
#pragma unroll
    for (int i = 0; i < 3; ++i) o[i] = fma(R.m[3 * i + 2], v[2], fma(R.m[3 * i + 1], v[1], R.m[3 * i] * v[0]));
}
RDV_DEV void rot_apply_T(const Rot &R, const double v[3], double o[3])
{
#pragma unroll
    for (int i = 0; i < 3; ++i) o[i] = fma(R.m[6 + i], v[2], fma(R.m[3 + i], v[1], R.m[i] * v[0]));
}

#ifndef RDV_QUAT_ROTATE
#define RDV_QUAT_ROTATE 0
#endif
RDV_DEV void quat_rotate(const double q[4], const double v[3], double o[3])
{
    const double r = fast_rsqrt(dot4(q, q));
    const double w = q[0] * r, u[3] = {q[1] * r, q[2] * r, q[3] * r};
    double c[3], d[3];
    cross3(u, v, c);
    cross3(u, c, d);
#pragma unroll
    for (int i = 0; i < 3; ++i) o[i] = fma(2.0, fma(w, c[i], d[i]), v[i]);
}

RDV_DEV double fast_sqrt(double x) { return x > 0.0 ? x * fast_rsqrt(x) : 0.0; }

RDV_DEV double acos_of_rounded(double k)
{
    const double x0 = k * 1e-5;
    return acos(fma(fma(-x0, 1e5, k), 1e-5, x0));
}
#ifndef RDV_ACOS_TABLE
#define RDV_ACOS_TABLE 1
#endif
#ifndef RDV_TABLE_INT_INDEX
#define RDV_TABLE_INT_INDEX 0
#endif
constexpr int ACOS_TABLE_HALF = 100000;
#if RDV_ACOS_TABLE
__device__ double g_acos_table[2 * ACOS_TABLE_HALF + 1];
#endif
RDV_DEV double rounded_angle_from(double dot, double n1sq, double n2sq)
{
    const double c = dot * fast_rsqrt(n1sq * n2sq);
#if RDV_ACOS_TABLE && RDV_TABLE_INT_INDEX
    const int ki = __double2int_rn(c * 1e5);
    if ((unsigned)(ki + ACOS_TABLE_HALF) <= 2u * ACOS_TABLE_HALF && (ki != 0 || c == c))
        return g_acos_table[ki + ACOS_TABLE_HALF];
    return acos_of_rounded(rint(c * 1e5));
#else
    const double k = rint(c * 1e5);
#if RDV_ACOS_TABLE
    if (fabs(k) <= (double)ACOS_TABLE_HALF) return g_acos_table[(int)k + ACOS_TABLE_HALF];
#endif
    return acos_of_rounded(k);
#endif
}

struct BodyConst { const double *I, *Iinv, *tau; };

template <bool ISO>
RDV_DEV void attitude_rhs(const double *y, const double *hw_iso, const BodyConst &b, double *f)
{
    double r = fast_rsqrt(dot4(y, y));
    double h1, h2, h3;
    if (ISO) { h1 = hw_iso[0]; h2 = hw_iso[1]; h3 = hw_iso[2]; }
    else     { h1 = 0.5 * y[4]; h2 = 0.5 * y[5]; h3 = 0.5 * y[6]; }
    double g0 = -fma(h3, y[3], fma(h2, y[2], h1 * y[1]));
    double g1 = fma(-h2, y[3], fma(h3, y[2], h1 * y[0]));
    double g2 = fma(h1, y[3], fma(-h3, y[1], h2 * y[0]));
    double g3 = fma(-h1, y[2], fma(h2, y[1], h3 * y[0]));
    f[0] = g0 * r; f[1] = g1 * r; f[2] = g2 * r; f[3] = g3 * r;
    if (!ISO) {
        const double *w = y + 4;
        double L[3], c[3], t[3];
#pragma unroll
        for (int i = 0; i < 3; ++i) L[i] = fma(b.I[3 * i + 2], w[2], fma(b.I[3 * i + 1], w[1], b.I[3 * i] * w[0]));
        cross3(w, L, c);
#pragma unroll
        for (int i = 0; i < 3; ++i) t[i] = b.tau[i] - c[i];
#pragma unroll
        for (int i = 0; i < 3; ++i)
            f[4 + i] = fma(b.Iinv[3 * i + 2], t[2], fma(b.Iinv[3 * i + 1], t[1], b.Iinv[3 * i] * t[0]));
    }
}

#ifndef RDV_RK_CONST_BANK
#define RDV_RK_CONST_BANK 1
#endif
#if RDV_RK_CONST_BANK
__constant__ double c_rk[26] = {
    1.0 / 5,
    3.0 / 40,
    9.0 / 40,
    44.0 / 45,
    -56.0 / 15,
    32.0 / 9,
    19372.0 / 6561,
    -25360.0 / 2187,
    64448.0 / 6561,
    -212.0 / 729,
    9017.0 / 3168,
    -355.0 / 33,
    46732.0 / 5247,
    49.0 / 176,
    -5103.0 / 18656,
    35.0 / 384,
    500.0 / 1113,
    125.0 / 192,
    -2187.0 / 6784,
    11.0 / 84,
    -71.0 / 57600,
    71.0 / 16695,
    -71.0 / 1920,
    17253.0 / 339200,
    -22.0 / 525,
    1.0 / 40,
};
#define RK_A21 c_rk[0]
#define RK_A31 c_rk[1]
#define RK_A32 c_rk[2]
#define RK_A41 c_rk[3]
#define RK_A42 c_rk[4]
#define RK_A43 c_rk[5]
#define RK_A51 c_rk[6]
#define RK_A52 c_rk[7]
#define RK_A53 c_rk[8]
#define RK_A54 c_rk[9]
#define RK_A61 c_rk[10]
#define RK_A62 c_rk[11]
#define RK_A63 c_rk[12]
#define RK_A64 c_rk[13]
#define RK_A65 c_rk[14]
#define RK_B1 c_rk[15]
#define RK_B3 c_rk[16]
#define RK_B4 c_rk[17]
#define RK_B5 c_rk[18]
#define RK_B6 c_rk[19]
#define RK_E1 c_rk[20]
#define RK_E3 c_rk[21]
#define RK_E4 c_rk[22]
#define RK_E5 c_rk[23]
#define RK_E6 c_rk[24]
#define RK_E7 c_rk[25]
#else
#define RK_A21 (1.0 / 5)
#define RK_A31 (3.0 / 40)
#define RK_A32 (9.0 / 40)
#define RK_A41 (44.0 / 45)
#define RK_A42 (-56.0 / 15)
#define RK_A43 (32.0 / 9)
#define RK_A51 (19372.0 / 6561)
#define RK_A52 (-25360.0 / 2187)
#define RK_A53 (64448.0 / 6561)
#define RK_A54 (-212.0 / 729)
#define RK_A61 (9017.0 / 3168)
#define RK_A62 (-355.0 / 33)
#define RK_A63 (46732.0 / 5247)
#define RK_A64 (49.0 / 176)
#define RK_A65 (-5103.0 / 18656)
#define RK_B1 (35.0 / 384)
#define RK_B3 (500.0 / 1113)
#define RK_B4 (125.0 / 192)
#define RK_B5 (-2187.0 / 6784)
#define RK_B6 (11.0 / 84)
#define RK_E1 (-71.0 / 57600)
#define RK_E3 (71.0 / 16695)
#define RK_E4 (-71.0 / 1920)
#define RK_E5 (17253.0 / 339200)
#define RK_E6 (-22.0 / 525)
#define RK_E7 (1.0 / 40)
#endif
#define RK_RTOL 1e-7
#define RK_ATOL 1e-6

#ifndef RDV_CTRL_F32
#define RDV_CTRL_F32 1
#endif
RDV_DEV float rcp_f32(float x) { float r; asm("rcp.approx.ftz.f32 %0, %1;" : "=f"(r) : "f"(x)); return r; }
RDV_DEV float lg2_f32(float x) { float r; asm("lg2.approx.ftz.f32 %0, %1;" : "=f"(r) : "f"(x)); return r; }
RDV_DEV float ex2_f32(float x) { float r; asm("ex2.approx.ftz.f32 %0, %1;" : "=f"(r) : "f"(x)); return r; }
RDV_DEV float pow_neg_tenth_f32(float x) { return ex2_f32(-0.1f * lg2_f32(x)); }

#ifndef RDV_RK_INLINE
#define RDV_RK_INLINE 1
#endif
#if RDV_RK_INLINE
#define RDV_RK_FN RDV_DEV
#else
#define RDV_RK_FN __device__ __noinline__
#endif
template <bool ISO>
RDV_RK_FN int rk45_attitude(double (&y)[7], const double dt, const BodyConst &b, int &n_rejected)
{
    constexpr int NA = ISO ? 4 : 7;
    double hw[3] = {0.5 * y[4], 0.5 * y[5], 0.5 * y[6]};
    double K[7][NA];
    attitude_rhs<ISO>(y, hw, b, K[0]);

    double h_abs;
#if RDV_CTRL_F32
    {
        float inv_sc[7], d0s = 0.0f, d1s = 0.0f;
#pragma unroll
        for (int i = 0; i < 7; ++i) {
            const float yi = (float)y[i];
            inv_sc[i] = rcp_f32(fmaf(fabsf(yi), (float)RK_RTOL, (float)RK_ATOL));
            const float a = yi * inv_sc[i];
            d0s = fmaf(a, a, d0s);
        }
#pragma unroll
        for (int i = 0; i < NA; ++i) {
            const float a = (float)K[0][i] * inv_sc[i];
            d1s = fmaf(a, a, d1s);
        }
        d0s *= (1.0f / 7.0f);
        d1s *= (1.0f / 7.0f);
        float h0f;
        if (d0s < 1e-10f || d1s < 1e-10f) h0f = 1e-6f;
        else h0f = 0.01f * sqrtf(d0s * rcp_f32(d1s));
        const double h0 = fmin((double)h0f, dt);
        double y1[7], f1[NA];
#pragma unroll
        for (int i = 0; i < NA; ++i) y1[i] = fma(h0, K[0][i], y[i]);
#pragma unroll
        for (int i = NA; i < 7; ++i) y1[i] = y[i];
        attitude_rhs<ISO>(y1, hw, b, f1);
        float d2s = 0.0f;
#pragma unroll
        for (int i = 0; i < NA; ++i) {
            const float a = (float)(f1[i] - K[0][i]) * inv_sc[i];
            d2s = fmaf(a, a, d2s);
        }
        const float inv_h0 = rcp_f32((float)h0);
        d2s = d2s * (1.0f / 7.0f) * inv_h0 * inv_h0;
        float h1;
        if (d1s <= 1e-30f && d2s <= 1e-30f) h1 = fmaxf(1e-6f, (float)h0 * 1e-3f);
        else h1 = pow_neg_tenth_f32(fminf(fmaxf(d1s, d2s), 1e30f) * 1e4f);
        h_abs = fmin(fmin(100.0 * h0, (double)h1), dt);
    }
#else
    {
        double inv_sc[7], d0s = 0.0, d1s = 0.0;
#pragma unroll
        for (int i = 0; i < 7; ++i) {
            inv_sc[i] = fast_rcp(fma(fabs(y[i]), RK_RTOL, RK_ATOL));
            double a = y[i] * inv_sc[i];
            d0s = fma(a, a, d0s);
        }
#pragma unroll
        for (int i = 0; i < NA; ++i) {
            double a = K[0][i] * inv_sc[i];
            d1s = fma(a, a, d1s);
        }
        d0s *= (1.0 / 7.0);
        d1s *= (1.0 / 7.0);
        double h0;
        if (d0s < 1e-10 || d1s < 1e-10) h0 = 1e-6;
        else h0 = 0.01 * sqrt(d0s * fast_rcp(d1s));
        h0 = fmin(h0, dt);
        double y1[7], f1[NA];
#pragma unroll
        for (int i = 0; i < NA; ++i) y1[i] = fma(h0, K[0][i], y[i]);
#pragma unroll
        for (int i = NA; i < 7; ++i) y1[i] = y[i];
        attitude_rhs<ISO>(y1, hw, b, f1);
        double d2s = 0.0;
#pragma unroll
        for (int i = 0; i < NA; ++i) {
            double a = (f1[i] - K[0][i]) * inv_sc[i];
            d2s = fma(a, a, d2s);
        }
        double inv_h0 = fast_rcp(h0);
        d2s = d2s * (1.0 / 7.0) * inv_h0 * inv_h0;
        double h1;
        if (d1s <= 1e-30 && d2s <= 1e-30) h1 = fmax(1e-6, h0 * 1e-3);
        else h1 = pow_neg_tenth(fmax(d1s, d2s) * 1e4);
        h_abs = fmin(fmin(100.0 * h0, h1), dt);
    }
#endif

    double t = 0.0;
    int accepted = 0;
    for (;;) {
        const double min_step = 10.0 * (__longlong_as_double(__double_as_longlong(t) + 1) - t);
        if (h_abs < min_step) h_abs = min_step;
        bool rejected = false;
        double t_new, h;
        double y_new[NA];
        for (;;) {
            if (h_abs < min_step) return -1;
            t_new = t + h_abs;
            if (t_new - dt > 0.0) t_new = dt;
            h = t_new - t;
            h_abs = fabs(h);
            double ys[7];
            if (ISO) { ys[4] = y[4]; ys[5] = y[5]; ys[6] = y[6]; }
#pragma unroll
            for (int i = 0; i < NA; ++i) ys[i] = fma(K[0][i] * RK_A21, h, y[i]);
            attitude_rhs<ISO>(ys, hw, b, K[1]);
#pragma unroll
            for (int i = 0; i < NA; ++i) ys[i] = fma(fma(K[1][i], RK_A32, K[0][i] * RK_A31), h, y[i]);
            attitude_rhs<ISO>(ys, hw, b, K[2]);
#pragma unroll
            for (int i = 0; i < NA; ++i)
                ys[i] = fma(fma(K[2][i], RK_A43, fma(K[1][i], RK_A42, K[0][i] * RK_A41)), h, y[i]);
            attitude_rhs<ISO>(ys, hw, b, K[3]);
#pragma unroll
            for (int i = 0; i < NA; ++i)
                ys[i] = fma(fma(K[3][i], RK_A54, fma(K[2][i], RK_A53, fma(K[1][i], RK_A52, K[0][i] * RK_A51))), h,
                            y[i]);
            attitude_rhs<ISO>(ys, hw, b, K[4]);
#pragma unroll
            for (int i = 0; i < NA; ++i)
                ys[i] = fma(fma(K[4][i], RK_A65,
                                fma(K[3][i], RK_A64, fma(K[2][i], RK_A63, fma(K[1][i], RK_A62, K[0][i] * RK_A61)))),
                            h, y[i]);
            attitude_rhs<ISO>(ys, hw, b, K[5]);
#pragma unroll
            for (int i = 0; i < NA; ++i)
                ys[i] = fma(h,
                            fma(K[5][i], RK_B6,
                                fma(K[4][i], RK_B5, fma(K[3][i], RK_B4, fma(K[2][i], RK_B3, K[0][i] * RK_B1)))),
                            y[i]);
            attitude_rhs<ISO>(ys, hw, b, K[6]);
#pragma unroll
            for (int i = 0; i < NA; ++i) y_new[i] = ys[i];
            double eh[NA];
#pragma unroll
            for (int i = 0; i < NA; ++i)
                eh[i] = h * fma(K[6][i], RK_E7,
                                fma(K[5][i], RK_E6,
                                    fma(K[4][i], RK_E5, fma(K[3][i], RK_E4, fma(K[2][i], RK_E3, K[0][i] * RK_E1)))));
#if RDV_CTRL_F32
            float esf = 0.0f;
#pragma unroll
            for (int i = 0; i < NA; ++i) {
                const float m = (float)fmax(fabs(y[i]), fabs(y_new[i]));
                const float q = (float)eh[i] * rcp_f32(fmaf(m, (float)RK_RTOL, (float)RK_ATOL));
                esf = fmaf(q, q, esf);
            }
            esf *= (1.0f / 7.0f);
            if (!(esf < 1.0e30f)) return -1;
            bool accept = esf < 1.0f;
            if (fabsf(esf - 1.0f) < 1.0e-3f) {
                double es = 0.0;
#pragma unroll
                for (int i = 0; i < NA; ++i) {
                    const double e = eh[i] * fast_rcp(fma(fmax(fabs(y[i]), fabs(y_new[i])), RK_RTOL, RK_ATOL));
                    es = fma(e, e, es);
                }
                accept = es * (1.0 / 7.0) < 1.0;
            }
            const float p = 0.9f * pow_neg_tenth_f32(fminf(fmaxf(esf, 1e-12f), 1e8f));
            if (accept) {
                float factor = fminf(10.0f, p);
                if (rejected) factor = fminf(1.0f, factor);
                h_abs *= (double)factor;
                break;
            }
            h_abs *= (double)fmaxf(0.2f, p);
            rejected = true;
            ++n_rejected;
#else
            double es = 0.0;
#pragma unroll
            for (int i = 0; i < NA; ++i) {
                const double e = eh[i] * fast_rcp(fma(fmax(fabs(y[i]), fabs(y_new[i])), RK_RTOL, RK_ATOL));
                es = fma(e, e, es);
            }
            es *= (1.0 / 7.0);
            if (!(es < 1.0e300)) return -1;
            if (es < 1.0) {
                double factor = (es < 3.0e-11) ? 10.0 : fmin(10.0, 0.9 * pow_neg_tenth(es));
                if (rejected) factor = fmin(1.0, factor);
                h_abs *= factor;
                break;
            }
            h_abs *= (es > 1.0e7) ? 0.2 : fmax(0.2, 0.9 * pow_neg_tenth(es));
            rejected = true;
            ++n_rejected;
#endif
        }
        ++accepted;
        t = t_new;
#pragma unroll
        for (int i = 0; i < NA; ++i) { y[i] = y_new[i]; K[0][i] = K[6][i]; }
        if (t - dt >= 0.0) return accepted;
    }
}

RDV_DEV void rhs_plane(const double a, const double b, const double om2, double &ka, double &kb)
{
    const double t = om2 * b;
    const double g = fast_rsqrt(fma(t, b, a * a));
    ka = -(t * g);
    kb = a * g;
}

RDV_DEV float plane_err2_f32(const double ea, const double eb, const double a_new, const double b_new,
                             const float (&q0f)[4], const float (&pf)[4], const float (&ycf)[4], float (&ynf)[4])
{
    const float eaf = (float)ea, ebf = (float)eb, anf = (float)a_new, bnf = (float)b_new;
    float esf = 0.0f;
#pragma unroll
    for (int i = 0; i < 4; ++i) {
        ynf[i] = fmaf(bnf, pf[i], anf * q0f[i]);
        const float e = fmaf(ebf, pf[i], eaf * q0f[i]);
        const float m = fmaxf(fabsf(ycf[i]), fabsf(ynf[i]));
        const float q = e * rcp_f32(fmaf(m, (float)RK_RTOL, (float)RK_ATOL));
        esf = fmaf(q, q, esf);
    }
    return esf * (1.0f / 7.0f);
}
RDV_DEV double plane_err2_f64(const double ea, const double eb, const double a, const double b, const double a_new,
                              const double b_new, const double (&q0)[4], const double (&p)[4])
{
    double es = 0.0;
#pragma unroll
    for (int i = 0; i < 4; ++i) {
        const double yc = fma(b, p[i], a * q0[i]), yn = fma(b_new, p[i], a_new * q0[i]);
        const double e = fma(eb, p[i], ea * q0[i]) * fast_rcp(fma(fmax(fabs(yc), fabs(yn)), RK_RTOL, RK_ATOL));
        es = fma(e, e, es);
    }
    return es * (1.0 / 7.0);
}
#ifndef RDV_INIT_LAZY_D0
#define RDV_INIT_LAZY_D0 1
#endif
#ifndef RDV_INIT_NOSQRT
#define RDV_INIT_NOSQRT 1
#endif
#if RDV_INIT_LAZY_D0
RDV_DEV double plane_initial_step(const double (&y)[7], const float (&q0f)[4], const float (&pf)[4], const double om2,
                                  const double dt)
{
    float inv_sc[4], d0r = 0.0f, d1s = 0.0f;
#pragma unroll
    for (int i = 0; i < 4; ++i) {
        inv_sc[i] = rcp_f32(fmaf(fabsf(q0f[i]), (float)RK_RTOL, (float)RK_ATOL));
        const float v = q0f[i] * inv_sc[i], f = pf[i] * inv_sc[i];
        d0r = fmaf(v, v, d0r);
        d1s = fmaf(f, f, d1s);
    }
    const float d0q = d0r * (1.0f / 7.0f);
    d1s *= (1.0f / 7.0f);
    const float dtf = (float)dt;
#if RDV_INIT_NOSQRT
    const float om2f = (float)om2, room = fmaf(-0.5f * dtf, om2f, 0.975f);
    const bool d2_small = room > 0.0f && om2f * om2f * d0q <= d1s * room * room;
#else
    const float ub = (float)om2 * fmaf(0.5f * dtf, sqrtf(d1s), sqrtf(d0q));
    const bool d2_small = ub * ub * 1.05f <= d1s;
#endif
    if (d0q >= 1e-10f && d1s >= 1e-10f && d2_small) {
        const float h1 = pow_neg_tenth_f32(fminf(d1s, 1e30f) * 1e4f);
        const float lim = fminf(h1, dtf);
        if (d0q >= lim * lim * d1s * 1.0001f) return fmin((double)h1, dt);
    }
    float d0s = d0r;
#pragma unroll
    for (int i = 4; i < 7; ++i) {
        const float yi = (float)y[i];
        const float v = yi * rcp_f32(fmaf(fabsf(yi), (float)RK_RTOL, (float)RK_ATOL));
        d0s = fmaf(v, v, d0s);
    }
    d0s *= (1.0f / 7.0f);
    float h0f;
    if (d0s < 1e-10f || d1s < 1e-10f) h0f = 1e-6f;
    else h0f = 0.01f * sqrtf(d0s * rcp_f32(d1s));
    const double h0 = fmin((double)h0f, dt);
    const float h0c = (float)h0;
    const float ub2 = (float)om2 * fmaf(0.5f * h0c, sqrtf(d1s), sqrtf(d0q));
    float dmax = d1s;
    if (!(ub2 * ub2 * 1.05f <= d1s)) {
        double ka1, kb1;
        rhs_plane(1.0, h0, om2, ka1, kb1);
        const float daf = (float)ka1, dbf = (float)(kb1 - 1.0);
        float d2s = 0.0f;
#pragma unroll
        for (int i = 0; i < 4; ++i) {
            const float v = fmaf(dbf, pf[i], daf * q0f[i]) * inv_sc[i];
            d2s = fmaf(v, v, d2s);
        }
        const float inv_h0 = rcp_f32(h0c);
        d2s = d2s * (1.0f / 7.0f) * inv_h0 * inv_h0;
        dmax = fmaxf(d1s, d2s);
    }
    float h1;
    if (dmax <= 1e-30f) h1 = fmaxf(1e-6f, h0c * 1e-3f);
    else h1 = pow_neg_tenth_f32(fminf(dmax, 1e30f) * 1e4f);
    return fmin(fmin(100.0 * h0, (double)h1), dt);
}
#else
RDV_DEV double plane_initial_step(const double (&y)[7], const float (&q0f)[4], const float (&pf)[4], const double om2,
                                  const double dt)
{
    float inv_sc[4], d0s = 0.0f, d1s = 0.0f;
#pragma unroll
    for (int i = 0; i < 4; ++i) {
        inv_sc[i] = rcp_f32(fmaf(fabsf(q0f[i]), (float)RK_RTOL, (float)RK_ATOL));
        const float v = q0f[i] * inv_sc[i], f = pf[i] * inv_sc[i];
        d0s = fmaf(v, v, d0s);
        d1s = fmaf(f, f, d1s);
    }
    const float d0q = d0s * (1.0f / 7.0f);
#pragma unroll
    for (int i = 4; i < 7; ++i) {
        const float yi = (float)y[i];
        const float v = yi * rcp_f32(fmaf(fabsf(yi), (float)RK_RTOL, (float)RK_ATOL));
        d0s = fmaf(v, v, d0s);
    }
    d0s *= (1.0f / 7.0f);
    d1s *= (1.0f / 7.0f);
    float h0f;
    if (d0s < 1e-10f || d1s < 1e-10f) h0f = 1e-6f;
    else h0f = 0.01f * sqrtf(d0s * rcp_f32(d1s));
    const double h0 = fmin((double)h0f, dt);
    const float h0c = (float)h0;
    const float ub = (float)om2 * fmaf(0.5f * h0c, sqrtf(d1s), sqrtf(d0q));
    float dmax = d1s;
    if (!(ub * ub * 1.05f <= d1s)) {
        double ka1, kb1;
        rhs_plane(1.0, h0, om2, ka1, kb1);
        const float daf = (float)ka1, dbf = (float)(kb1 - 1.0);
        float d2s = 0.0f;
#pragma unroll
        for (int i = 0; i < 4; ++i) {
            const float v = fmaf(dbf, pf[i], daf * q0f[i]) * inv_sc[i];
            d2s = fmaf(v, v, d2s);
        }
        const float inv_h0 = rcp_f32(h0c);
        d2s = d2s * (1.0f / 7.0f) * inv_h0 * inv_h0;
        dmax = fmaxf(d1s, d2s);
    }
    float h1;
    if (dmax <= 1e-30f) h1 = fmaxf(1e-6f, h0c * 1e-3f);
    else h1 = pow_neg_tenth_f32(fminf(dmax, 1e30f) * 1e4f);
    return fmin(fmin(100.0 * h0, (double)h1), dt);
}
#endif

RDV_DEV void plane_basis(const double (&y)[7], double (&q0)[4], double (&p)[4], double &om2)
{
#pragma unroll
    for (int i = 0; i < 4; ++i) q0[i] = y[i];
    const double hs = 0.5 * fast_rsqrt(dot4(q0, q0));
    const double hw[3] = {hs * y[4], hs * y[5], hs * y[6]};
    p[0] = -fma(hw[2], q0[3], fma(hw[1], q0[2], hw[0] * q0[1]));
    p[1] = fma(-hw[1], q0[3], fma(hw[2], q0[2], hw[0] * q0[0]));
    p[2] = fma(hw[0], q0[3], fma(-hw[2], q0[1], hw[1] * q0[0]));
    p[3] = fma(-hw[0], q0[2], fma(hw[1], q0[1], hw[2] * q0[0]));
    om2 = fma(hw[2], hw[2], fma(hw[1], hw[1], hw[0] * hw[0]));
}

struct PlanePoint { double a, b, ka, kb, t; float yf[4]; };

#ifndef RDV_RK_PINGPONG
#define RDV_RK_PINGPONG 0
#endif
#ifndef RDV_MERGE_RARE
#define RDV_MERGE_RARE 1
#endif
#ifndef RDV_LATE_MINSTEP
#define RDV_LATE_MINSTEP 0
#endif
#ifndef RDV_LAZY_MINSTEP
#define RDV_LAZY_MINSTEP 0
#endif
#ifndef RDV_LAST_FLAG
#define RDV_LAST_FLAG 0
#endif
#ifndef RDV_LAST_SHORTCUT
#define RDV_LAST_SHORTCUT 1
#endif
RDV_DEV int plane_step(const PlanePoint &s, PlanePoint &n, double &h_abs, int &n_rejected, const double om2, const double dt,
                        const double (&q0)[4], const double (&p)[4], const float (&q0f)[4], const float (&pf)[4])
{
    const double a = s.a, b = s.b, t = s.t;
#if RDV_LAZY_MINSTEP
    const double lazy_thr = dt * 1e-13;
    if (h_abs < lazy_thr) {
        const double min_step = 10.0 * (__longlong_as_double(__double_as_longlong(t) + 1) - t);
        if (h_abs < min_step) h_abs = min_step;
    }
#else
    const double min_step = 10.0 * (__longlong_as_double(__double_as_longlong(t) + 1) - t);
    if (h_abs < min_step) h_abs = min_step;
#endif
    bool rejected = false;
    for (;;) {
#if !RDV_LATE_MINSTEP && !RDV_LAZY_MINSTEP
        if (h_abs < min_step) return 0;
#endif
        double t_new = t + h_abs;
#if RDV_LAST_FLAG || RDV_LAST_SHORTCUT
        const double over = t_new - dt;
        if (over > 0.0) t_new = dt;
        const bool last = over >= 0.0;
#else
        if (t_new - dt > 0.0) t_new = dt;
#endif
        const double h = t_new - t;
        h_abs = fabs(h);
        double ka[7], kb[7], as, bs;
        ka[0] = s.ka; kb[0] = s.kb;
        as = fma(ka[0] * RK_A21, h, a);
        bs = fma(kb[0] * RK_A21, h, b);
        rhs_plane(as, bs, om2, ka[1], kb[1]);
        as = fma(fma(ka[1], RK_A32, ka[0] * RK_A31), h, a);
        bs = fma(fma(kb[1], RK_A32, kb[0] * RK_A31), h, b);
        rhs_plane(as, bs, om2, ka[2], kb[2]);
        as = fma(fma(ka[2], RK_A43, fma(ka[1], RK_A42, ka[0] * RK_A41)), h, a);
        bs = fma(fma(kb[2], RK_A43, fma(kb[1], RK_A42, kb[0] * RK_A41)), h, b);
        rhs_plane(as, bs, om2, ka[3], kb[3]);
        as = fma(fma(ka[3], RK_A54, fma(ka[2], RK_A53, fma(ka[1], RK_A52, ka[0] * RK_A51))), h, a);
        bs = fma(fma(kb[3], RK_A54, fma(kb[2], RK_A53, fma(kb[1], RK_A52, kb[0] * RK_A51))), h, b);
        rhs_plane(as, bs, om2, ka[4], kb[4]);
        as = fma(fma(ka[4], RK_A65, fma(ka[3], RK_A64, fma(ka[2], RK_A63, fma(ka[1], RK_A62, ka[0] * RK_A61)))), h, a);
        bs = fma(fma(kb[4], RK_A65, fma(kb[3], RK_A64, fma(kb[2], RK_A63, fma(kb[1], RK_A62, kb[0] * RK_A61)))), h, b);
        rhs_plane(as, bs, om2, ka[5], kb[5]);
        const double a_new = fma(h, fma(ka[5], RK_B6, fma(ka[4], RK_B5, fma(ka[3], RK_B4, fma(ka[2], RK_B3, ka[0] * RK_B1)))), a);
        const double b_new = fma(h, fma(kb[5], RK_B6, fma(kb[4], RK_B5, fma(kb[3], RK_B4, fma(kb[2], RK_B3, kb[0] * RK_B1)))), b);
        rhs_plane(a_new, b_new, om2, ka[6], kb[6]);
        const double ea = h * fma(ka[6], RK_E7, fma(ka[5], RK_E6, fma(ka[4], RK_E5, fma(ka[3], RK_E4,
                              fma(ka[2], RK_E3, ka[0] * RK_E1)))));
        const double eb = h * fma(kb[6], RK_E7, fma(kb[5], RK_E6, fma(kb[4], RK_E5, fma(kb[3], RK_E4,
                              fma(kb[2], RK_E3, kb[0] * RK_E1)))));
#if RDV_LAST_SHORTCUT
        if (last) {
            const float eaf = (float)ea, ebf = (float)eb;
            float nq = 0.0f, np = 0.0f;
#pragma unroll
            for (int i = 0; i < 4; ++i) { nq = fmaf(q0f[i], q0f[i], nq); np = fmaf(pf[i], pf[i], np); }
            const float ub = fmaf(eaf * eaf, nq, ebf * ebf * np) * (2.0f / 7.0f * 1.0e12f);
            if (ub < 0.99f) {
                n.a = a_new; n.b = b_new; n.ka = ka[6]; n.kb = kb[6]; n.t = t_new;
                return 2;
            }
        }
#endif
        const float esf = plane_err2_f32(ea, eb, a_new, b_new, q0f, pf, s.yf, n.yf);
#if RDV_MERGE_RARE
        bool accept = esf < 1.0f;
        if (!(fabsf(esf - 1.0f) >= 1.0e-3f && esf < 1.0e30f)) {
            if (!(esf < 1.0e30f)) return 0;
            accept = plane_err2_f64(ea, eb, a, b, a_new, b_new, q0, p) < 1.0;
        }
#else
        if (!(esf < 1.0e30f)) return 0;
        bool accept = esf < 1.0f;
        if (fabsf(esf - 1.0f) < 1.0e-3f)
            accept = plane_err2_f64(ea, eb, a, b, a_new, b_new, q0, p) < 1.0;
#endif
        const float pw = 0.9f * pow_neg_tenth_f32(fminf(fmaxf(esf, 1e-12f), 1e8f));
        if (accept) {
            float factor = fminf(10.0f, pw);
            if (rejected) factor = fminf(1.0f, factor);
            h_abs *= (double)factor;
            n.a = a_new; n.b = b_new; n.ka = ka[6]; n.kb = kb[6]; n.t = t_new;
#if RDV_LAST_FLAG || RDV_LAST_SHORTCUT
            return last ? 2 : 1;
#else
            return 1;
#endif
        }
        h_abs *= (double)fmaxf(0.2f, pw);
        rejected = true;
        ++n_rejected;
#if RDV_LAZY_MINSTEP
        if (h_abs < lazy_thr) {
            const double min_step = 10.0 * (__longlong_as_double(__double_as_longlong(t) + 1) - t);
            if (h_abs < min_step) return 0;
        }
#elif RDV_LATE_MINSTEP
        if (h_abs < min_step) return 0;
#endif
    }
}

#ifndef RDV_NO_REMAT
#define RDV_NO_REMAT 1
#endif
#if RDV_NO_REMAT
#define RDV_KEEP_F32(x) asm volatile("" : "+f"(x))
#else
#define RDV_KEEP_F32(x)
#endif
RDV_RK_FN int rk45_iso_plane(double (&y)[7], const double dt, int &n_rejected)
{
    double q0[4], p[4], om2;
    plane_basis(y, q0, p, om2);
    float q0f[4], pf[4];
    PlanePoint X, Y;
#pragma unroll
    for (int i = 0; i < 4; ++i) {
        q0f[i] = (float)q0[i]; pf[i] = (float)p[i];
        RDV_KEEP_F32(q0f[i]); RDV_KEEP_F32(pf[i]);
        X.yf[i] = q0f[i];
    }
    X.a = 1.0; X.b = 0.0; X.ka = 0.0; X.kb = 1.0; X.t = 0.0;
    double h_abs = plane_initial_step(y, q0f, pf, om2, dt);
    int accepted = 0;
#if RDV_RK_PINGPONG
    for (;;) {
        if (!plane_step(X, Y, h_abs, n_rejected, om2, dt, q0, p, q0f, pf)) return -1;
        ++accepted;
        if (Y.t - dt >= 0.0) { X.a = Y.a; X.b = Y.b; break; }
        if (!plane_step(Y, X, h_abs, n_rejected, om2, dt, q0, p, q0f, pf)) return -1;
        ++accepted;
        if (X.t - dt >= 0.0) break;
    }
#else
    for (;;) {
        const int r = plane_step(X, Y, h_abs, n_rejected, om2, dt, q0, p, q0f, pf);
        if (!r) return -1;
        ++accepted;
        X = Y;
#if RDV_LAST_FLAG || RDV_LAST_SHORTCUT
        if (r == 2) break;
#else
        if (X.t - dt >= 0.0) break;
#endif
    }
#endif
#pragma unroll
    for (int i = 0; i < 4; ++i) y[i] = fma(X.b, p[i], X.a * q0[i]);
    return accepted;
}

RDV_DEV int rk45_iso_plane_pair(double (&ya)[7], double (&yb)[7], const double dt, int &n_rejected)
{
    double q0[2][4], p[2][4], om2[2], a[2], b[2], ka0[2], kb0[2], h_abs[2], t[2];
    float q0f[2][4], pf[2][4], ycf[2][4];
    int accepted[2] = {0, 0};
    bool done[2] = {false, false}, rejected[2] = {false, false}, failed[2] = {false, false};
    plane_basis(ya, q0[0], p[0], om2[0]);
    plane_basis(yb, q0[1], p[1], om2[1]);
#pragma unroll
    for (int c = 0; c < 2; ++c) {
        a[c] = 1.0; b[c] = 0.0; ka0[c] = 0.0; kb0[c] = 1.0;
#pragma unroll
        for (int i = 0; i < 4; ++i) { q0f[c][i] = (float)q0[c][i]; pf[c][i] = (float)p[c][i]; ycf[c][i] = q0f[c][i]; }
    }
    h_abs[0] = plane_initial_step(ya, q0f[0], pf[0], om2[0], dt);
    h_abs[1] = plane_initial_step(yb, q0f[1], pf[1], om2[1], dt);
    t[0] = t[1] = 0.0;
    while (!((done[0] || failed[0]) && (done[1] || failed[1]))) {
        double h[2], t_new[2], ha[2], as[2], bs[2];
        bool fail_now[2];
        double ka1[2], kb1[2], ka2[2], kb2[2], ka3[2], kb3[2], ka4[2], kb4[2], ka5[2], kb5[2], ka6[2], kb6[2];
#pragma unroll
        for (int c = 0; c < 2; ++c) {
            const double min_step = 10.0 * (__longlong_as_double(__double_as_longlong(t[c]) + 1) - t[c]);
            fail_now[c] = rejected[c] && h_abs[c] < min_step;
            ha[c] = rejected[c] ? h_abs[c] : fmax(h_abs[c], min_step);
            t_new[c] = t[c] + ha[c];
            if (t_new[c] - dt > 0.0) t_new[c] = dt;
            h[c] = t_new[c] - t[c];
            ha[c] = fabs(h[c]);
        }
#define RDV_PSTAGE(KA, KB, EA, EB)                                                       \
        _Pragma("unroll") for (int c = 0; c < 2; ++c) { as[c] = (EA); bs[c] = (EB); }    \
        _Pragma("unroll") for (int c = 0; c < 2; ++c) rhs_plane(as[c], bs[c], om2[c], KA[c], KB[c]);
        RDV_PSTAGE(ka1, kb1, fma(ka0[c] * RK_A21, h[c], a[c]), fma(kb0[c] * RK_A21, h[c], b[c]))
        RDV_PSTAGE(ka2, kb2, fma(fma(ka1[c], RK_A32, ka0[c] * RK_A31), h[c], a[c]),
                   fma(fma(kb1[c], RK_A32, kb0[c] * RK_A31), h[c], b[c]))
        RDV_PSTAGE(ka3, kb3, fma(fma(ka2[c], RK_A43, fma(ka1[c], RK_A42, ka0[c] * RK_A41)), h[c], a[c]),
                   fma(fma(kb2[c], RK_A43, fma(kb1[c], RK_A42, kb0[c] * RK_A41)), h[c], b[c]))
        RDV_PSTAGE(ka4, kb4,
                   fma(fma(ka3[c], RK_A54, fma(ka2[c], RK_A53, fma(ka1[c], RK_A52, ka0[c] * RK_A51))), h[c], a[c]),
                   fma(fma(kb3[c], RK_A54, fma(kb2[c], RK_A53, fma(kb1[c], RK_A52, kb0[c] * RK_A51))), h[c], b[c]))
        RDV_PSTAGE(ka5, kb5,
                   fma(fma(ka4[c], RK_A65, fma(ka3[c], RK_A64, fma(ka2[c], RK_A63, fma(ka1[c], RK_A62, ka0[c] * RK_A61)))),
                       h[c], a[c]),
                   fma(fma(kb4[c], RK_A65, fma(kb3[c], RK_A64, fma(kb2[c], RK_A63, fma(kb1[c], RK_A62, kb0[c] * RK_A61)))),
                       h[c], b[c]))
        RDV_PSTAGE(ka6, kb6,
                   fma(h[c], fma(ka5[c], RK_B6, fma(ka4[c], RK_B5, fma(ka3[c], RK_B4, fma(ka2[c], RK_B3, ka0[c] * RK_B1)))),
                       a[c]),
                   fma(h[c], fma(kb5[c], RK_B6, fma(kb4[c], RK_B5, fma(kb3[c], RK_B4, fma(kb2[c], RK_B3, kb0[c] * RK_B1)))),
                       b[c]))
#undef RDV_PSTAGE
#pragma unroll
        for (int c = 0; c < 2; ++c) {
            const double ea = h[c] * fma(ka6[c], RK_E7, fma(ka5[c], RK_E6, fma(ka4[c], RK_E5, fma(ka3[c], RK_E4,
                                     fma(ka2[c], RK_E3, ka0[c] * RK_E1)))));
            const double eb = h[c] * fma(kb6[c], RK_E7, fma(kb5[c], RK_E6, fma(kb4[c], RK_E5, fma(kb3[c], RK_E4,
                                     fma(kb2[c], RK_E3, kb0[c] * RK_E1)))));
            float ynf[4];
            const float esf = plane_err2_f32(ea, eb, as[c], bs[c], q0f[c], pf[c], ycf[c], ynf);
            const bool live = !done[c] && !failed[c];
            const bool bad = fail_now[c] || !(esf < 1.0e30f);
            bool accept = esf < 1.0f;
            if (fabsf(esf - 1.0f) < 1.0e-3f)
                accept = plane_err2_f64(ea, eb, a[c], b[c], as[c], bs[c], q0[c], p[c]) < 1.0;
            const float pw = 0.9f * pow_neg_tenth_f32(fminf(fmaxf(esf, 1e-12f), 1e8f));
            float factor = accept ? fminf(10.0f, pw) : fmaxf(0.2f, pw);
            if (accept && rejected[c]) factor = fminf(1.0f, factor);
            const bool commit = live && !bad && accept;
            if (live) {
                failed[c] = bad;
                h_abs[c] = bad ? h_abs[c] : ha[c] * (double)factor;
                rejected[c] = !accept;
                n_rejected += (!bad && !accept) ? 1 : 0;
            }
            if (commit) {
                a[c] = as[c]; b[c] = bs[c]; ka0[c] = ka6[c]; kb0[c] = kb6[c];
#pragma unroll
                for (int i = 0; i < 4; ++i) ycf[c][i] = ynf[i];
                t[c] = t_new[c];
                accepted[c] += 1;
                done[c] = t_new[c] - dt >= 0.0;
            }
        }
    }
#pragma unroll
    for (int i = 0; i < 4; ++i) {
        ya[i] = fma(b[0], p[0][i], a[0] * q0[0][i]);
        yb[i] = fma(b[1], p[1][i], a[1] * q0[1][i]);
    }
    return (failed[0] || failed[1]) ? -1 : accepted[0] + accepted[1];
}

RDV_DEV void closed_form_attitude(double (&y)[7], const double dt)
{
    double wsq = fma(y[6], y[6], fma(y[5], y[5], y[4] * y[4]));
    if (wsq == 0.0) return;
    double rq = fast_rsqrt(dot4(y, y));
    double wn = sqrt(wsq);
    double s, c;
    sincos(0.5 * wn * dt * rq, &s, &c);
    double k = s / wn;
    double g0 = -fma(y[6], y[3], fma(y[5], y[2], y[4] * y[1]));
    double g1 = fma(-y[5], y[3], fma(y[6], y[2], y[4] * y[0]));
    double g2 = fma(y[4], y[3], fma(-y[6], y[1], y[5] * y[0]));
    double g3 = fma(-y[4], y[2], fma(y[5], y[1], y[6] * y[0]));
    y[0] = fma(g0, k, y[0] * c); y[1] = fma(g1, k, y[1] * c);
    y[2] = fma(g2, k, y[2] * c); y[3] = fma(g3, k, y[3] * c);
}

RDV_DEV void philox4x32_10(uint32_t (&c)[4], uint32_t k0, uint32_t k1)
{
#pragma unroll
    for (int r = 0; r < 10; ++r) {
        uint32_t hi0 = __umulhi(0xD2511F53u, c[0]), lo0 = 0xD2511F53u * c[0];
        uint32_t hi1 = __umulhi(0xCD9E8D57u, c[2]), lo1 = 0xCD9E8D57u * c[2];
        uint32_t n0 = hi1 ^ c[1] ^ k0, n2 = hi0 ^ c[3] ^ k1;
        c[0] = n0; c[1] = lo1; c[2] = n2; c[3] = lo0;
        k0 += 0x9E3779B9u; k1 += 0xBB67AE85u;
    }
}
RDV_DEV void philox_uniform_pair(uint64_t seed, int64_t env_id, int32_t episode, uint32_t blk, double &u0,
                                 double &u1)
{
    uint32_t c[4] = {(uint32_t)env_id, (uint32_t)((uint64_t)env_id >> 32), (uint32_t)episode, blk};
    philox4x32_10(c, (uint32_t)seed, (uint32_t)(seed >> 32));
    u0 = ((double)(c[0] >> 5) * 67108864.0 + (double)(c[1] >> 6)) * (1.0 / 9007199254740992.0);
    u1 = ((double)(c[2] >> 5) * 67108864.0 + (double)(c[3] >> 6)) * (1.0 / 9007199254740992.0);
}

}
```

Baseline: 6.564 billion.

## Replace plane RK45 stage evaluations with fitted polynomial step map

Within a rotation-plane step, the Dormand-Prince attempt is replaced by closed-form polynomials in x = (h g)^2 om2. These give the new state and error estimate directly instead of seven rhs evaluations, each with an rsqrt. A stored g per plane point replaces the carried FSAL derivatives. A coverage check routes states outside the fitted range to the original stagewise solver through noinline fallbacks. The aim is to cut the FP64 arithmetic per attempt, at the cost of relying on fitted coefficients that must match the RK45 map closely enough to keep acceptance behaviour and results unchanged.

```diff
diff --git a/reinforcement_learning_rendezvous_b200/_native.py b/reinforcement_learning_rendezvous_b200/_native.py
--- a/reinforcement_learning_rendezvous_b200/_native.py
+++ b/reinforcement_learning_rendezvous_b200/_native.py
@@ -14,7 +14,7 @@
 HOST_SRC = os.path.join(CSRC_DIR, "rdv_host.c")
 HOST_LIB = os.path.join(PKG_DIR, "_rdv_host" + (sysconfig.get_config_var("EXT_SUFFIX") or ".so"))
 SOURCES = ("rdv_b200.cu",)
-HEADERS = ("rdv_math.cuh", "rdv_env.cuh", "rdv_step.cuh", "rdv_policy.cuh", "rdv_policy_tc.cuh")
+HEADERS = ("rdv_math.cuh", "rdv_plane_poly.h", "rdv_env.cuh", "rdv_step.cuh", "rdv_policy.cuh", "rdv_policy_tc.cuh")
 
 ABI_VERSION = 15
 OBS_DIM, ACT_DIM, N_UNIFORMS = 17, 6, 24
diff --git a/reinforcement_learning_rendezvous_b200/csrc/rdv_b200.cu b/reinforcement_learning_rendezvous_b200/csrc/rdv_b200.cu
--- a/reinforcement_learning_rendezvous_b200/csrc/rdv_b200.cu
+++ b/reinforcement_learning_rendezvous_b200/csrc/rdv_b200.cu
@@ -1001,7 +1001,20 @@
         case 2: r = fast_sqrt(v); break;
         case 3: r = pow_neg_tenth(v); break;
         case 4: r = (double)pow_neg_tenth_f32((float)v); break;
-        default: r = rounded_angle_from(v, 1.0, 1.0); break;
+        case 5: r = rounded_angle_from(v, 1.0, 1.0); break;
+        default: {
+            double P, Q, R, I;
+            if (op < 10) {
+                plane_poly(v, P, Q, R, I);
+            } else {
+                const double h = sqrt(v);
+                plane_attempt<false>(1.0, 0.0, 1.0, 1.0, h, P, Q, R, I);
+                Q /= h; R /= v * v * v; I /= h * v * v;
+            }
+            const int k = (op - 6) & 3;
+            r = k == 0 ? P : k == 1 ? Q : k == 2 ? R : I;
+            break;
+        }
     }
     y[i] = r;
 }
@@ -1505,7 +1518,7 @@
 int rdv_math_probe(const double *x, double *y, int64_t n, int op, void *cuda_stream)
 {
     if (!x || !y) return RDV_ERR_NULL;
-    if (n < 0 || op < 0 || op > 5) return RDV_ERR_SIZE;
+    if (n < 0 || op < 0 || op > 13) return RDV_ERR_SIZE;
     if (n == 0) return RDV_OK;
     if (!ensure_tables((cudaStream_t)cuda_stream)) return RDV_ERR_CUDA;
     math_probe_kernel<<<(unsigned)((n + 255) / 256), 256, 0, (cudaStream_t)cuda_stream>>>(x, y, n, op);
diff --git a/reinforcement_learning_rendezvous_b200/csrc/rdv_math.cuh b/reinforcement_learning_rendezvous_b200/csrc/rdv_math.cuh
--- a/reinforcement_learning_rendezvous_b200/csrc/rdv_math.cuh
+++ b/reinforcement_learning_rendezvous_b200/csrc/rdv_math.cuh
@@ -2,6 +2,7 @@
 #include <cuda_runtime.h>
 #include <stdint.h>
 #include "rdv_b200.h"
+#include "rdv_plane_poly.h"
 
 #define RDV_DEV __device__ __forceinline__
 
@@ -475,214 +476,53 @@
     ka = -(t * g);
     kb = a * g;
 }
-
-RDV_DEV float plane_err2_f32(const double ea, const double eb, const double a_new, const double b_new,
-                             const float (&q0f)[4], const float (&pf)[4], const float (&ycf)[4], float (&ynf)[4])
-{
-    const float eaf = (float)ea, ebf = (float)eb, anf = (float)a_new, bnf = (float)b_new;
-    float esf = 0.0f;
-#pragma unroll
-    for (int i = 0; i < 4; ++i) {
-        ynf[i] = fmaf(bnf, pf[i], anf * q0f[i]);
-        const float e = fmaf(ebf, pf[i], eaf * q0f[i]);
-        const float m = fmaxf(fabsf(ycf[i]), fabsf(ynf[i]));
-        const float q = e * rcp_f32(fmaf(m, (float)RK_RTOL, (float)RK_ATOL));
-        esf = fmaf(q, q, esf);
-    }
-    return esf * (1.0f / 7.0f);
-}
-RDV_DEV double plane_err2_f64(const double ea, const double eb, const double a, const double b, const double a_new,
-                              const double b_new, const double (&q0)[4], const double (&p)[4])
-{
-    double es = 0.0;
-#pragma unroll
-    for (int i = 0; i < 4; ++i) {
-        const double yc = fma(b, p[i], a * q0[i]), yn = fma(b_new, p[i], a_new * q0[i]);
-        const double e = fma(eb, p[i], ea * q0[i]) * fast_rcp(fma(fmax(fabs(yc), fabs(yn)), RK_RTOL, RK_ATOL));
-        es = fma(e, e, es);
-    }
-    return es * (1.0 / 7.0);
-}
-#ifndef RDV_INIT_LAZY_D0
-#define RDV_INIT_LAZY_D0 1
-#endif
-#ifndef RDV_INIT_NOSQRT
-#define RDV_INIT_NOSQRT 1
-#endif
-#if RDV_INIT_LAZY_D0
-RDV_DEV double plane_initial_step(const double (&y)[7], const float (&q0f)[4], const float (&pf)[4], const double om2,
-                                  const double dt)
-{
-    float inv_sc[4], d0r = 0.0f, d1s = 0.0f;
-#pragma unroll
-    for (int i = 0; i < 4; ++i) {
-        inv_sc[i] = rcp_f32(fmaf(fabsf(q0f[i]), (float)RK_RTOL, (float)RK_ATOL));
-        const float v = q0f[i] * inv_sc[i], f = pf[i] * inv_sc[i];
-        d0r = fmaf(v, v, d0r);
-        d1s = fmaf(f, f, d1s);
-    }
-    const float d0q = d0r * (1.0f / 7.0f);
-    d1s *= (1.0f / 7.0f);
-    const float dtf = (float)dt;
-#if RDV_INIT_NOSQRT
-    const float om2f = (float)om2, room = fmaf(-0.5f * dtf, om2f, 0.975f);
-    const bool d2_small = room > 0.0f && om2f * om2f * d0q <= d1s * room * room;
-#else
-    const float ub = (float)om2 * fmaf(0.5f * dtf, sqrtf(d1s), sqrtf(d0q));
-    const bool d2_small = ub * ub * 1.05f <= d1s;
-#endif
-    if (d0q >= 1e-10f && d1s >= 1e-10f && d2_small) {
-        const float h1 = pow_neg_tenth_f32(fminf(d1s, 1e30f) * 1e4f);
-        const float lim = fminf(h1, dtf);
-        if (d0q >= lim * lim * d1s * 1.0001f) return fmin((double)h1, dt);
-    }
-    float d0s = d0r;
-#pragma unroll
-    for (int i = 4; i < 7; ++i) {
-        const float yi = (float)y[i];
-        const float v = yi * rcp_f32(fmaf(fabsf(yi), (float)RK_RTOL, (float)RK_ATOL));
-        d0s = fmaf(v, v, d0s);
-    }
-    d0s *= (1.0f / 7.0f);
-    float h0f;
-    if (d0s < 1e-10f || d1s < 1e-10f) h0f = 1e-6f;
-    else h0f = 0.01f * sqrtf(d0s * rcp_f32(d1s));
-    const double h0 = fmin((double)h0f, dt);
-    const float h0c = (float)h0;
-    const float ub2 = (float)om2 * fmaf(0.5f * h0c, sqrtf(d1s), sqrtf(d0q));
-    float dmax = d1s;
-    if (!(ub2 * ub2 * 1.05f <= d1s)) {
-        double ka1, kb1;
-        rhs_plane(1.0, h0, om2, ka1, kb1);
-        const float daf = (float)ka1, dbf = (float)(kb1 - 1.0);
-        float d2s = 0.0f;
-#pragma unroll
-        for (int i = 0; i < 4; ++i) {
-            const float v = fmaf(dbf, pf[i], daf * q0f[i]) * inv_sc[i];
-            d2s = fmaf(v, v, d2s);
-        }
-        const float inv_h0 = rcp_f32(h0c);
-        d2s = d2s * (1.0f / 7.0f) * inv_h0 * inv_h0;
-        dmax = fmaxf(d1s, d2s);
-    }
-    float h1;
-    if (dmax <= 1e-30f) h1 = fmaxf(1e-6f, h0c * 1e-3f);
-    else h1 = pow_neg_tenth_f32(fminf(dmax, 1e30f) * 1e4f);
-    return fmin(fmin(100.0 * h0, (double)h1), dt);
-}
-#else
-RDV_DEV double plane_initial_step(const double (&y)[7], const float (&q0f)[4], const float (&pf)[4], const double om2,
-                                  const double dt)
-{
-    float inv_sc[4], d0s = 0.0f, d1s = 0.0f;
-#pragma unroll
-    for (int i = 0; i < 4; ++i) {
-        inv_sc[i] = rcp_f32(fmaf(fabsf(q0f[i]), (float)RK_RTOL, (float)RK_ATOL));
-        const float v = q0f[i] * inv_sc[i], f = pf[i] * inv_sc[i];
-        d0s = fmaf(v, v, d0s);
-        d1s = fmaf(f, f, d1s);
-    }
-    const float d0q = d0s * (1.0f / 7.0f);
-#pragma unroll
-    for (int i = 4; i < 7; ++i) {
-        const float yi = (float)y[i];
-        const float v = yi * rcp_f32(fmaf(fabsf(yi), (float)RK_RTOL, (float)RK_ATOL));
-        d0s = fmaf(v, v, d0s);
-    }
-    d0s *= (1.0f / 7.0f);
-    d1s *= (1.0f / 7.0f);
-    float h0f;
-    if (d0s < 1e-10f || d1s < 1e-10f) h0f = 1e-6f;
-    else h0f = 0.01f * sqrtf(d0s * rcp_f32(d1s));
-    const double h0 = fmin((double)h0f, dt);
-    const float h0c = (float)h0;
-    const float ub = (float)om2 * fmaf(0.5f * h0c, sqrtf(d1s), sqrtf(d0q));
-    float dmax = d1s;
-    if (!(ub * ub * 1.05f <= d1s)) {
-        double ka1, kb1;
-        rhs_plane(1.0, h0, om2, ka1, kb1);
-        const float daf = (float)ka1, dbf = (float)(kb1 - 1.0);
-        float d2s = 0.0f;
-#pragma unroll
-        for (int i = 0; i < 4; ++i) {
-            const float v = fmaf(dbf, pf[i], daf * q0f[i]) * inv_sc[i];
-            d2s = fmaf(v, v, d2s);
-        }
-        const float inv_h0 = rcp_f32(h0c);
-        d2s = d2s * (1.0f / 7.0f) * inv_h0 * inv_h0;
-        dmax = fmaxf(d1s, d2s);
-    }
-    float h1;
-    if (dmax <= 1e-30f) h1 = fmaxf(1e-6f, h0c * 1e-3f);
-    else h1 = pow_neg_tenth_f32(fminf(dmax, 1e30f) * 1e4f);
-    return fmin(fmin(100.0 * h0, (double)h1), dt);
-}
-#endif
-
-RDV_DEV void plane_basis(const double (&y)[7], double (&q0)[4], double (&p)[4], double &om2)
-{
-#pragma unroll
-    for (int i = 0; i < 4; ++i) q0[i] = y[i];
-    const double hs = 0.5 * fast_rsqrt(dot4(q0, q0));
-    const double hw[3] = {hs * y[4], hs * y[5], hs * y[6]};
-    p[0] = -fma(hw[2], q0[3], fma(hw[1], q0[2], hw[0] * q0[1]));
-    p[1] = fma(-hw[1], q0[3], fma(hw[2], q0[2], hw[0] * q0[0]));
-    p[2] = fma(hw[0], q0[3], fma(-hw[2], q0[1], hw[1] * q0[0]));
-    p[3] = fma(-hw[0], q0[2], fma(hw[1], q0[1], hw[2] * q0[0]));
-    om2 = fma(hw[2], hw[2], fma(hw[1], hw[1], hw[0] * hw[0]));
-}
-
-struct PlanePoint { double a, b, ka, kb, t; float yf[4]; };
-
-#ifndef RDV_RK_PINGPONG
-#define RDV_RK_PINGPONG 0
-#endif
-#ifndef RDV_MERGE_RARE
-#define RDV_MERGE_RARE 1
-#endif
-#ifndef RDV_LATE_MINSTEP
-#define RDV_LATE_MINSTEP 0
-#endif
-#ifndef RDV_LAZY_MINSTEP
-#define RDV_LAZY_MINSTEP 0
-#endif
-#ifndef RDV_LAST_FLAG
-#define RDV_LAST_FLAG 0
-#endif
-#ifndef RDV_LAST_SHORTCUT
-#define RDV_LAST_SHORTCUT 1
-#endif
-RDV_DEV int plane_step(const PlanePoint &s, PlanePoint &n, double &h_abs, int &n_rejected, const double om2, const double dt,
-                        const double (&q0)[4], const double (&p)[4], const float (&q0f)[4], const float (&pf)[4])
-{
-    const double a = s.a, b = s.b, t = s.t;
-#if RDV_LAZY_MINSTEP
-    const double lazy_thr = dt * 1e-13;
-    if (h_abs < lazy_thr) {
-        const double min_step = 10.0 * (__longlong_as_double(__double_as_longlong(t) + 1) - t);
-        if (h_abs < min_step) h_abs = min_step;
-    }
-#else
-    const double min_step = 10.0 * (__longlong_as_double(__double_as_longlong(t) + 1) - t);
-    if (h_abs < min_step) h_abs = min_step;
-#endif
-    bool rejected = false;
-    for (;;) {
-#if !RDV_LATE_MINSTEP && !RDV_LAZY_MINSTEP
-        if (h_abs < min_step) return 0;
-#endif
-        double t_new = t + h_abs;
-#if RDV_LAST_FLAG || RDV_LAST_SHORTCUT
-        const double over = t_new - dt;
-        if (over > 0.0) t_new = dt;
-        const bool last = over >= 0.0;
-#else
-        if (t_new - dt > 0.0) t_new = dt;
-#endif
-        const double h = t_new - t;
-        h_abs = fabs(h);
+RDV_DEV double plane_g(const double a, const double b, const double om2) { return fast_rsqrt(fma(om2 * b, b, a * a)); }
+
+#ifndef RDV_PLANE_POLY
+#define RDV_PLANE_POLY 1
+#endif
+constexpr int PP_P1 = 0, PP_Q1 = PP_P1 + RDV_PP_N_P1, PP_R = PP_Q1 + RDV_PP_N_Q1, PP_I = PP_R + RDV_PP_N_R;
+__constant__ double c_pp[PP_I + RDV_PP_N_I] = {RDV_PP_P1, RDV_PP_Q1, RDV_PP_R, RDV_PP_I};
+
+template <int OFF, int N>
+RDV_DEV double pp_horner(const double x)
+{
+    double r = c_pp[OFF + N - 1];
+#pragma unroll
+    for (int k = N - 2; k >= 0; --k) r = fma(r, x, c_pp[OFF + k]);
+    return r;
+}
+RDV_DEV void plane_poly(const double x, double &P, double &Q, double &R, double &I)
+{
+    P = fma(x, pp_horner<PP_P1, RDV_PP_N_P1>(x), 1.0);
+    Q = fma(x, pp_horner<PP_Q1, RDV_PP_N_Q1>(x), 1.0);
+    R = pp_horner<PP_R, RDV_PP_N_R>(x);
+    I = pp_horner<PP_I, RDV_PP_N_I>(x);
+}
+RDV_DEV bool plane_poly_covers(const double (&y)[7], const double dt)
+{
+    const double w2 = fma(y[6], y[6], fma(y[5], y[5], y[4] * y[4]));
+    const double q2 = fma(y[3], y[3], fma(y[2], y[2], fma(y[1], y[1], y[0] * y[0])));
+    return 0.25 * w2 * (dt * dt) <= (RDV_PP_X_MAX * (1.0 - 0x1p-20)) * q2;
+}
+
+template <bool POLY>
+RDV_DEV void plane_attempt(const double a, const double b, const double g, const double om2, const double h,
+                           double &a_new, double &b_new, double &ea, double &eb)
+{
+    if (POLY) {
+        const double hg = h * g, t = hg * om2;
+        const double u = hg * a, v = t * b, x = t * hg;
+        double P, Q, R, I;
+        plane_poly(x, P, Q, R, I);
+        a_new = fma(a, P, -(v * Q));
+        b_new = fma(b, P, u * Q);
+        const double x2 = x * x, xr = x * R;
+        ea = x2 * fma(a, xr, -(v * I));
+        eb = x2 * fma(b, xr, u * I);
+    } else {
         double ka[7], kb[7], as, bs;
-        ka[0] = s.ka; kb[0] = s.kb;
+        ka[0] = -((om2 * b) * g); kb[0] = a * g;
         as = fma(ka[0] * RK_A21, h, a);
         bs = fma(kb[0] * RK_A21, h, b);
         rhs_plane(as, bs, om2, ka[1], kb[1]);
@@ -698,13 +538,222 @@
         as = fma(fma(ka[4], RK_A65, fma(ka[3], RK_A64, fma(ka[2], RK_A63, fma(ka[1], RK_A62, ka[0] * RK_A61)))), h, a);
         bs = fma(fma(kb[4], RK_A65, fma(kb[3], RK_A64, fma(kb[2], RK_A63, fma(kb[1], RK_A62, kb[0] * RK_A61)))), h, b);
         rhs_plane(as, bs, om2, ka[5], kb[5]);
-        const double a_new = fma(h, fma(ka[5], RK_B6, fma(ka[4], RK_B5, fma(ka[3], RK_B4, fma(ka[2], RK_B3, ka[0] * RK_B1)))), a);
-        const double b_new = fma(h, fma(kb[5], RK_B6, fma(kb[4], RK_B5, fma(kb[3], RK_B4, fma(kb[2], RK_B3, kb[0] * RK_B1)))), b);
+        a_new = fma(h, fma(ka[5], RK_B6, fma(ka[4], RK_B5, fma(ka[3], RK_B4, fma(ka[2], RK_B3, ka[0] * RK_B1)))), a);
+        b_new = fma(h, fma(kb[5], RK_B6, fma(kb[4], RK_B5, fma(kb[3], RK_B4, fma(kb[2], RK_B3, kb[0] * RK_B1)))), b);
         rhs_plane(a_new, b_new, om2, ka[6], kb[6]);
-        const double ea = h * fma(ka[6], RK_E7, fma(ka[5], RK_E6, fma(ka[4], RK_E5, fma(ka[3], RK_E4,
-                              fma(ka[2], RK_E3, ka[0] * RK_E1)))));
-        const double eb = h * fma(kb[6], RK_E7, fma(kb[5], RK_E6, fma(kb[4], RK_E5, fma(kb[3], RK_E4,
-                              fma(kb[2], RK_E3, kb[0] * RK_E1)))));
+        ea = h * fma(ka[6], RK_E7, fma(ka[5], RK_E6, fma(ka[4], RK_E5, fma(ka[3], RK_E4, fma(ka[2], RK_E3, ka[0] * RK_E1)))));
+        eb = h * fma(kb[6], RK_E7, fma(kb[5], RK_E6, fma(kb[4], RK_E5, fma(kb[3], RK_E4, fma(kb[2], RK_E3, kb[0] * RK_E1)))));
+    }
+}
+
+RDV_DEV float plane_err2_f32(const double ea, const double eb, const double a_new, const double b_new,
+                             const float (&q0f)[4], const float (&pf)[4], const float (&ycf)[4], float (&ynf)[4])
+{
+    const float eaf = (float)ea, ebf = (float)eb, anf = (float)a_new, bnf = (float)b_new;
+    float esf = 0.0f;
+#pragma unroll
+    for (int i = 0; i < 4; ++i) {
+        ynf[i] = fmaf(bnf, pf[i], anf * q0f[i]);
+        const float e = fmaf(ebf, pf[i], eaf * q0f[i]);
+        const float m = fmaxf(fabsf(ycf[i]), fabsf(ynf[i]));
+        const float q = e * rcp_f32(fmaf(m, (float)RK_RTOL, (float)RK_ATOL));
+        esf = fmaf(q, q, esf);
+    }
+    return esf * (1.0f / 7.0f);
+}
+RDV_DEV double plane_err2_f64(const double ea, const double eb, const double a, const double b, const double a_new,
+                              const double b_new, const double (&q0)[4], const double (&p)[4])
+{
+    double es = 0.0;
+#pragma unroll
+    for (int i = 0; i < 4; ++i) {
+        const double yc = fma(b, p[i], a * q0[i]), yn = fma(b_new, p[i], a_new * q0[i]);
+        const double e = fma(eb, p[i], ea * q0[i]) * fast_rcp(fma(fmax(fabs(yc), fabs(yn)), RK_RTOL, RK_ATOL));
+        es = fma(e, e, es);
+    }
+    return es * (1.0 / 7.0);
+}
+#ifndef RDV_INIT_LAZY_D0
+#define RDV_INIT_LAZY_D0 1
+#endif
+#ifndef RDV_INIT_NOSQRT
+#define RDV_INIT_NOSQRT 1
+#endif
+#if RDV_INIT_LAZY_D0
+RDV_DEV double plane_initial_step(const double (&y)[7], const float (&q0f)[4], const float (&pf)[4], const double om2,
+                                  const double dt)
+{
+    float inv_sc[4], d0r = 0.0f, d1s = 0.0f;
+#pragma unroll
+    for (int i = 0; i < 4; ++i) {
+        inv_sc[i] = rcp_f32(fmaf(fabsf(q0f[i]), (float)RK_RTOL, (float)RK_ATOL));
+        const float v = q0f[i] * inv_sc[i], f = pf[i] * inv_sc[i];
+        d0r = fmaf(v, v, d0r);
+        d1s = fmaf(f, f, d1s);
+    }
+    const float d0q = d0r * (1.0f / 7.0f);
+    d1s *= (1.0f / 7.0f);
+    const float dtf = (float)dt;
+#if RDV_INIT_NOSQRT
+    const float om2f = (float)om2, room = fmaf(-0.5f * dtf, om2f, 0.975f);
+    const bool d2_small = room > 0.0f && om2f * om2f * d0q <= d1s * room * room;
+#else
+    const float ub = (float)om2 * fmaf(0.5f * dtf, sqrtf(d1s), sqrtf(d0q));
+    const bool d2_small = ub * ub * 1.05f <= d1s;
+#endif
+    if (d0q >= 1e-10f && d1s >= 1e-10f && d2_small) {
+        const float h1 = pow_neg_tenth_f32(fminf(d1s, 1e30f) * 1e4f);
+        const float lim = fminf(h1, dtf);
+        if (d0q >= lim * lim * d1s * 1.0001f) return fmin((double)h1, dt);
+    }
+    float d0s = d0r;
+#pragma unroll
+    for (int i = 4; i < 7; ++i) {
+        const float yi = (float)y[i];
+        const float v = yi * rcp_f32(fmaf(fabsf(yi), (float)RK_RTOL, (float)RK_ATOL));
+        d0s = fmaf(v, v, d0s);
+    }
+    d0s *= (1.0f / 7.0f);
+    float h0f;
+    if (d0s < 1e-10f || d1s < 1e-10f) h0f = 1e-6f;
+    else h0f = 0.01f * sqrtf(d0s * rcp_f32(d1s));
+    const double h0 = fmin((double)h0f, dt);
+    const float h0c = (float)h0;
+    const float ub2 = (float)om2 * fmaf(0.5f * h0c, sqrtf(d1s), sqrtf(d0q));
+    float dmax = d1s;
+    if (!(ub2 * ub2 * 1.05f <= d1s)) {
+        double ka1, kb1;
+        rhs_plane(1.0, h0, om2, ka1, kb1);
+        const float daf = (float)ka1, dbf = (float)(kb1 - 1.0);
+        float d2s = 0.0f;
+#pragma unroll
+        for (int i = 0; i < 4; ++i) {
+            const float v = fmaf(dbf, pf[i], daf * q0f[i]) * inv_sc[i];
+            d2s = fmaf(v, v, d2s);
+        }
+        const float inv_h0 = rcp_f32(h0c);
+        d2s = d2s * (1.0f / 7.0f) * inv_h0 * inv_h0;
+        dmax = fmaxf(d1s, d2s);
+    }
+    float h1;
+    if (dmax <= 1e-30f) h1 = fmaxf(1e-6f, h0c * 1e-3f);
+    else h1 = pow_neg_tenth_f32(fminf(dmax, 1e30f) * 1e4f);
+    return fmin(fmin(100.0 * h0, (double)h1), dt);
+}
+#else
+RDV_DEV double plane_initial_step(const double (&y)[7], const float (&q0f)[4], const float (&pf)[4], const double om2,
+                                  const double dt)
+{
+    float inv_sc[4], d0s = 0.0f, d1s = 0.0f;
+#pragma unroll
+    for (int i = 0; i < 4; ++i) {
+        inv_sc[i] = rcp_f32(fmaf(fabsf(q0f[i]), (float)RK_RTOL, (float)RK_ATOL));
+        const float v = q0f[i] * inv_sc[i], f = pf[i] * inv_sc[i];
+        d0s = fmaf(v, v, d0s);
+        d1s = fmaf(f, f, d1s);
+    }
+    const float d0q = d0s * (1.0f / 7.0f);
+#pragma unroll
+    for (int i = 4; i < 7; ++i) {
+        const float yi = (float)y[i];
+        const float v = yi * rcp_f32(fmaf(fabsf(yi), (float)RK_RTOL, (float)RK_ATOL));
+        d0s = fmaf(v, v, d0s);
+    }
+    d0s *= (1.0f / 7.0f);
+    d1s *= (1.0f / 7.0f);
+    float h0f;
+    if (d0s < 1e-10f || d1s < 1e-10f) h0f = 1e-6f;
+    else h0f = 0.01f * sqrtf(d0s * rcp_f32(d1s));
+    const double h0 = fmin((double)h0f, dt);
+    const float h0c = (float)h0;
+    const float ub = (float)om2 * fmaf(0.5f * h0c, sqrtf(d1s), sqrtf(d0q));
+    float dmax = d1s;
+    if (!(ub * ub * 1.05f <= d1s)) {
+        double ka1, kb1;
+        rhs_plane(1.0, h0, om2, ka1, kb1);
+        const float daf = (float)ka1, dbf = (float)(kb1 - 1.0);
+        float d2s = 0.0f;
+#pragma unroll
+        for (int i = 0; i < 4; ++i) {
+            const float v = fmaf(dbf, pf[i], daf * q0f[i]) * inv_sc[i];
+            d2s = fmaf(v, v, d2s);
+        }
+        const float inv_h0 = rcp_f32(h0c);
+        d2s = d2s * (1.0f / 7.0f) * inv_h0 * inv_h0;
+        dmax = fmaxf(d1s, d2s);
+    }
+    float h1;
+    if (dmax <= 1e-30f) h1 = fmaxf(1e-6f, h0c * 1e-3f);
+    else h1 = pow_neg_tenth_f32(fminf(dmax, 1e30f) * 1e4f);
+    return fmin(fmin(100.0 * h0, (double)h1), dt);
+}
+#endif
+
+RDV_DEV void plane_basis(const double (&y)[7], double (&q0)[4], double (&p)[4], double &om2)
+{
+#pragma unroll
+    for (int i = 0; i < 4; ++i) q0[i] = y[i];
+    const double hs = 0.5 * fast_rsqrt(dot4(q0, q0));
+    const double hw[3] = {hs * y[4], hs * y[5], hs * y[6]};
+    p[0] = -fma(hw[2], q0[3], fma(hw[1], q0[2], hw[0] * q0[1]));
+    p[1] = fma(-hw[1], q0[3], fma(hw[2], q0[2], hw[0] * q0[0]));
+    p[2] = fma(hw[0], q0[3], fma(-hw[2], q0[1], hw[1] * q0[0]));
+    p[3] = fma(-hw[0], q0[2], fma(hw[1], q0[1], hw[2] * q0[0]));
+    om2 = fma(hw[2], hw[2], fma(hw[1], hw[1], hw[0] * hw[0]));
+}
+
+struct PlanePoint { double a, b, g, t; float yf[4]; };
+
+#ifndef RDV_RK_PINGPONG
+#define RDV_RK_PINGPONG 0
+#endif
+#ifndef RDV_MERGE_RARE
+#define RDV_MERGE_RARE 1
+#endif
+#ifndef RDV_LATE_MINSTEP
+#define RDV_LATE_MINSTEP 0
+#endif
+#ifndef RDV_LAZY_MINSTEP
+#define RDV_LAZY_MINSTEP 0
+#endif
+#ifndef RDV_LAST_FLAG
+#define RDV_LAST_FLAG 0
+#endif
+#ifndef RDV_LAST_SHORTCUT
+#define RDV_LAST_SHORTCUT 1
+#endif
+template <bool POLY>
+RDV_DEV int plane_step(const PlanePoint &s, PlanePoint &n, double &h_abs, int &n_rejected, const double om2, const double dt,
+                        const double (&q0)[4], const double (&p)[4], const float (&q0f)[4], const float (&pf)[4])
+{
+    const double a = s.a, b = s.b, t = s.t;
+#if RDV_LAZY_MINSTEP
+    const double lazy_thr = dt * 1e-13;
+    if (h_abs < lazy_thr) {
+        const double min_step = 10.0 * (__longlong_as_double(__double_as_longlong(t) + 1) - t);
+        if (h_abs < min_step) h_abs = min_step;
+    }
+#else
+    const double min_step = 10.0 * (__longlong_as_double(__double_as_longlong(t) + 1) - t);
+    if (h_abs < min_step) h_abs = min_step;
+#endif
+    bool rejected = false;
+    for (;;) {
+#if !RDV_LATE_MINSTEP && !RDV_LAZY_MINSTEP
+        if (h_abs < min_step) return 0;
+#endif
+        double t_new = t + h_abs;
+#if RDV_LAST_FLAG || RDV_LAST_SHORTCUT
+        const double over = t_new - dt;
+        if (over > 0.0) t_new = dt;
+        const bool last = over >= 0.0;
+#else
+        if (t_new - dt > 0.0) t_new = dt;
+#endif
+        const double h = t_new - t;
+        h_abs = fabs(h);
+        double a_new, b_new, ea, eb;
+        plane_attempt<POLY>(a, b, s.g, om2, h, a_new, b_new, ea, eb);
 #if RDV_LAST_SHORTCUT
         if (last) {
             const float eaf = (float)ea, ebf = (float)eb;
@@ -713,7 +762,7 @@
             for (int i = 0; i < 4; ++i) { nq = fmaf(q0f[i], q0f[i], nq); np = fmaf(pf[i], pf[i], np); }
             const float ub = fmaf(eaf * eaf, nq, ebf * ebf * np) * (2.0f / 7.0f * 1.0e12f);
             if (ub < 0.99f) {
-                n.a = a_new; n.b = b_new; n.ka = ka[6]; n.kb = kb[6]; n.t = t_new;
+                n.a = a_new; n.b = b_new; n.t = t_new;
                 return 2;
             }
         }
@@ -736,7 +785,7 @@
             float factor = fminf(10.0f, pw);
             if (rejected) factor = fminf(1.0f, factor);
             h_abs *= (double)factor;
-            n.a = a_new; n.b = b_new; n.ka = ka[6]; n.kb = kb[6]; n.t = t_new;
+            n.a = a_new; n.b = b_new; n.g = plane_g(a_new, b_new, om2); n.t = t_new;
 #if RDV_LAST_FLAG || RDV_LAST_SHORTCUT
             return last ? 2 : 1;
 #else
@@ -765,7 +814,8 @@
 #else
 #define RDV_KEEP_F32(x)
 #endif
-RDV_RK_FN int rk45_iso_plane(double (&y)[7], const double dt, int &n_rejected)
+template <bool POLY>
+RDV_DEV int rk45_iso_plane_solve(double (&y)[7], const double dt, int &n_rejected)
 {
     double q0[4], p[4], om2;
     plane_basis(y, q0, p, om2);
@@ -777,21 +827,21 @@
         RDV_KEEP_F32(q0f[i]); RDV_KEEP_F32(pf[i]);
         X.yf[i] = q0f[i];
     }
-    X.a = 1.0; X.b = 0.0; X.ka = 0.0; X.kb = 1.0; X.t = 0.0;
+    X.a = 1.0; X.b = 0.0; X.g = 1.0; X.t = 0.0;
     double h_abs = plane_initial_step(y, q0f, pf, om2, dt);
     int accepted = 0;
 #if RDV_RK_PINGPONG
     for (;;) {
-        if (!plane_step(X, Y, h_abs, n_rejected, om2, dt, q0, p, q0f, pf)) return -1;
+        if (!plane_step<POLY>(X, Y, h_abs, n_rejected, om2, dt, q0, p, q0f, pf)) return -1;
         ++accepted;
         if (Y.t - dt >= 0.0) { X.a = Y.a; X.b = Y.b; break; }
-        if (!plane_step(Y, X, h_abs, n_rejected, om2, dt, q0, p, q0f, pf)) return -1;
+        if (!plane_step<POLY>(Y, X, h_abs, n_rejected, om2, dt, q0, p, q0f, pf)) return -1;
         ++accepted;
         if (X.t - dt >= 0.0) break;
     }
 #else
     for (;;) {
-        const int r = plane_step(X, Y, h_abs, n_rejected, om2, dt, q0, p, q0f, pf);
+        const int r = plane_step<POLY>(X, Y, h_abs, n_rejected, om2, dt, q0, p, q0f, pf);
         if (!r) return -1;
         ++accepted;
         X = Y;
@@ -806,10 +856,24 @@
     for (int i = 0; i < 4; ++i) y[i] = fma(X.b, p[i], X.a * q0[i]);
     return accepted;
 }
-
-RDV_DEV int rk45_iso_plane_pair(double (&ya)[7], double (&yb)[7], const double dt, int &n_rejected)
-{
-    double q0[2][4], p[2][4], om2[2], a[2], b[2], ka0[2], kb0[2], h_abs[2], t[2];
+__device__ __noinline__ int rk45_iso_plane_stagewise(double (&y)[7], const double dt, int &n_rejected)
+{
+    return rk45_iso_plane_solve<false>(y, dt, n_rejected);
+}
+RDV_RK_FN int rk45_iso_plane(double (&y)[7], const double dt, int &n_rejected)
+{
+#if RDV_PLANE_POLY
+    if (!plane_poly_covers(y, dt)) return rk45_iso_plane_stagewise(y, dt, n_rejected);
+    return rk45_iso_plane_solve<true>(y, dt, n_rejected);
+#else
+    return rk45_iso_plane_solve<false>(y, dt, n_rejected);
+#endif
+}
+
+template <bool POLY>
+RDV_DEV int rk45_iso_plane_pair_solve(double (&ya)[7], double (&yb)[7], const double dt, int &n_rejected)
+{
+    double q0[2][4], p[2][4], om2[2], a[2], b[2], g[2], h_abs[2], t[2];
     float q0f[2][4], pf[2][4], ycf[2][4];
     int accepted[2] = {0, 0};
     bool done[2] = {false, false}, rejected[2] = {false, false}, failed[2] = {false, false};
@@ -817,7 +881,7 @@
     plane_basis(yb, q0[1], p[1], om2[1]);
 #pragma unroll
     for (int c = 0; c < 2; ++c) {
-        a[c] = 1.0; b[c] = 0.0; ka0[c] = 0.0; kb0[c] = 1.0;
+        a[c] = 1.0; b[c] = 0.0; g[c] = 1.0;
 #pragma unroll
         for (int i = 0; i < 4; ++i) { q0f[c][i] = (float)q0[c][i]; pf[c][i] = (float)p[c][i]; ycf[c][i] = q0f[c][i]; }
     }
@@ -825,9 +889,8 @@
     h_abs[1] = plane_initial_step(yb, q0f[1], pf[1], om2[1], dt);
     t[0] = t[1] = 0.0;
     while (!((done[0] || failed[0]) && (done[1] || failed[1]))) {
-        double h[2], t_new[2], ha[2], as[2], bs[2];
+        double h[2], t_new[2], ha[2], as[2], bs[2], ea[2], eb[2];
         bool fail_now[2];
-        double ka1[2], kb1[2], ka2[2], kb2[2], ka3[2], kb3[2], ka4[2], kb4[2], ka5[2], kb5[2], ka6[2], kb6[2];
 #pragma unroll
         for (int c = 0; c < 2; ++c) {
             const double min_step = 10.0 * (__longlong_as_double(__double_as_longlong(t[c]) + 1) - t[c]);
@@ -838,41 +901,17 @@
             h[c] = t_new[c] - t[c];
             ha[c] = fabs(h[c]);
         }
-#define RDV_PSTAGE(KA, KB, EA, EB)                                                       \
-        _Pragma("unroll") for (int c = 0; c < 2; ++c) { as[c] = (EA); bs[c] = (EB); }    \
-        _Pragma("unroll") for (int c = 0; c < 2; ++c) rhs_plane(as[c], bs[c], om2[c], KA[c], KB[c]);
-        RDV_PSTAGE(ka1, kb1, fma(ka0[c] * RK_A21, h[c], a[c]), fma(kb0[c] * RK_A21, h[c], b[c]))
-        RDV_PSTAGE(ka2, kb2, fma(fma(ka1[c], RK_A32, ka0[c] * RK_A31), h[c], a[c]),
-                   fma(fma(kb1[c], RK_A32, kb0[c] * RK_A31), h[c], b[c]))
-        RDV_PSTAGE(ka3, kb3, fma(fma(ka2[c], RK_A43, fma(ka1[c], RK_A42, ka0[c] * RK_A41)), h[c], a[c]),
-                   fma(fma(kb2[c], RK_A43, fma(kb1[c], RK_A42, kb0[c] * RK_A41)), h[c], b[c]))
-        RDV_PSTAGE(ka4, kb4,
-                   fma(fma(ka3[c], RK_A54, fma(ka2[c], RK_A53, fma(ka1[c], RK_A52, ka0[c] * RK_A51))), h[c], a[c]),
-                   fma(fma(kb3[c], RK_A54, fma(kb2[c], RK_A53, fma(kb1[c], RK_A52, kb0[c] * RK_A51))), h[c], b[c]))
-        RDV_PSTAGE(ka5, kb5,
-                   fma(fma(ka4[c], RK_A65, fma(ka3[c], RK_A64, fma(ka2[c], RK_A63, fma(ka1[c], RK_A62, ka0[c] * RK_A61)))),
-                       h[c], a[c]),
-                   fma(fma(kb4[c], RK_A65, fma(kb3[c], RK_A64, fma(kb2[c], RK_A63, fma(kb1[c], RK_A62, kb0[c] * RK_A61)))),
-                       h[c], b[c]))
-        RDV_PSTAGE(ka6, kb6,
-                   fma(h[c], fma(ka5[c], RK_B6, fma(ka4[c], RK_B5, fma(ka3[c], RK_B4, fma(ka2[c], RK_B3, ka0[c] * RK_B1)))),
-                       a[c]),
-                   fma(h[c], fma(kb5[c], RK_B6, fma(kb4[c], RK_B5, fma(kb3[c], RK_B4, fma(kb2[c], RK_B3, kb0[c] * RK_B1)))),
-                       b[c]))
-#undef RDV_PSTAGE
+#pragma unroll
+        for (int c = 0; c < 2; ++c) plane_attempt<POLY>(a[c], b[c], g[c], om2[c], h[c], as[c], bs[c], ea[c], eb[c]);
 #pragma unroll
         for (int c = 0; c < 2; ++c) {
-            const double ea = h[c] * fma(ka6[c], RK_E7, fma(ka5[c], RK_E6, fma(ka4[c], RK_E5, fma(ka3[c], RK_E4,
-                                     fma(ka2[c], RK_E3, ka0[c] * RK_E1)))));
-            const double eb = h[c] * fma(kb6[c], RK_E7, fma(kb5[c], RK_E6, fma(kb4[c], RK_E5, fma(kb3[c], RK_E4,
-                                     fma(kb2[c], RK_E3, kb0[c] * RK_E1)))));
             float ynf[4];
-            const float esf = plane_err2_f32(ea, eb, as[c], bs[c], q0f[c], pf[c], ycf[c], ynf);
+            const float esf = plane_err2_f32(ea[c], eb[c], as[c], bs[c], q0f[c], pf[c], ycf[c], ynf);
             const bool live = !done[c] && !failed[c];
             const bool bad = fail_now[c] || !(esf < 1.0e30f);
             bool accept = esf < 1.0f;
             if (fabsf(esf - 1.0f) < 1.0e-3f)
-                accept = plane_err2_f64(ea, eb, a[c], b[c], as[c], bs[c], q0[c], p[c]) < 1.0;
+                accept = plane_err2_f64(ea[c], eb[c], a[c], b[c], as[c], bs[c], q0[c], p[c]) < 1.0;
             const float pw = 0.9f * pow_neg_tenth_f32(fminf(fmaxf(esf, 1e-12f), 1e8f));
             float factor = accept ? fminf(10.0f, pw) : fmaxf(0.2f, pw);
             if (accept && rejected[c]) factor = fminf(1.0f, factor);
@@ -884,7 +923,7 @@
                 n_rejected += (!bad && !accept) ? 1 : 0;
             }
             if (commit) {
-                a[c] = as[c]; b[c] = bs[c]; ka0[c] = ka6[c]; kb0[c] = kb6[c];
+                a[c] = as[c]; b[c] = bs[c]; g[c] = plane_g(as[c], bs[c], om2[c]);
 #pragma unroll
                 for (int i = 0; i < 4; ++i) ycf[c][i] = ynf[i];
                 t[c] = t_new[c];
@@ -899,6 +938,21 @@
         yb[i] = fma(b[1], p[1][i], a[1] * q0[1][i]);
     }
     return (failed[0] || failed[1]) ? -1 : accepted[0] + accepted[1];
+}
+__device__ __noinline__ int rk45_iso_plane_pair_mixed(double (&ya)[7], double (&yb)[7], const double dt, int &n_rejected)
+{
+    const int ka = rk45_iso_plane(ya, dt, n_rejected);
+    const int kb = rk45_iso_plane(yb, dt, n_rejected);
+    return (ka < 0 || kb < 0) ? -1 : ka + kb;
+}
+RDV_DEV int rk45_iso_plane_pair(double (&ya)[7], double (&yb)[7], const double dt, int &n_rejected)
+{
+#if RDV_PLANE_POLY
+    if (!(plane_poly_covers(ya, dt) && plane_poly_covers(yb, dt))) return rk45_iso_plane_pair_mixed(ya, yb, dt, n_rejected);
+    return rk45_iso_plane_pair_solve<true>(ya, yb, dt, n_rejected);
+#else
+    return rk45_iso_plane_pair_solve<false>(ya, yb, dt, n_rejected);
+#endif
 }
 
 RDV_DEV void closed_form_attitude(double (&y)[7], const double dt)
diff --git a/reinforcement_learning_rendezvous_b200/csrc/rdv_plane_poly.h b/reinforcement_learning_rendezvous_b200/csrc/rdv_plane_poly.h
--- /dev/null
+++ b/reinforcement_learning_rendezvous_b200/csrc/rdv_plane_poly.h
@@ -0,0 +1,12 @@
+#pragma once
+
+#define RDV_PP_X_MAX 0x1.0000000000000p-5
+#define RDV_PP_DRIFT_PER_S 0x1.baba499e5e7c4p-32
+#define RDV_PP_N_P1 6
+#define RDV_PP_N_Q1 6
+#define RDV_PP_N_R 6
+#define RDV_PP_N_I 7
+#define RDV_PP_P1 -0x1.0000000000000p-1, 0x1.55555555569c0p-5, -0x1.6c16c1a7b1e63p-10, 0x1.3a12eca2c202ap-13, 0x1.240b0be0712d1p-13, -0x1.3da83ecc050d1p-13
+#define RDV_PP_Q1 -0x1.5555555555556p-3, 0x1.1111111114115p-7, -0x1.0b9ce2a379badp-12, 0x1.06063e43fc2c0p-13, 0x1.99c5c856f8a9ep-13, -0x1.2b709d4815f18p-14
+#define RDV_PP_R 0x1.f77b5d5ab37c1p-13, -0x1.3b7e55f619a41p-12, 0x1.46a63835862c4p-14, -0x1.23e08ebdb3974p-15, 0x1.39583db11f396p-16, -0x1.d4b94627038a3p-18
+#define RDV_PP_I -0x1.6fa61c49a5a77p-17, 0x1.79b33de2ab462p-12, -0x1.6e1044fe3ed77p-13, 0x1.595b20d8dffbfp-15, -0x1.d56a8cec1ea20p-16, 0x1.6ec90da08237ap-17, -0x1.4c960ed2cffefp-18
```

Measured after the change: 6.844 billion, median of 6. 1.04x the previous value.
